# NERSC/swin_v2_weather

Hardware: AMD Instinct MI355X
Metric: ERA5 samples/sec (73x721x1440) swin_73var depth12 (higher is better)
Workload: dtype bf16

## Files before the change

include/swv2.h:

```cpp
#ifndef SWV2_H
#define SWV2_H
#include <stddef.h>
#include <stdint.h>

#ifdef __cplusplus
extern "C" {
#endif

#define SWV2_VERSION 113

enum {
    SWV2_OK = 0,
    SWV2_ERR_INVALID = -1,
    SWV2_ERR_UNSUPPORTED = -2,
    SWV2_ERR_LAUNCH = -3
};

int swv2_version(void);
const char* swv2_last_error(void);

int swv2_attn_geometry(int L, int head_dim, int* Lp, int* DP);

int swv2_attn_fwd_regime(int L, int head_dim, int has_bias, int dbg);

#define SWV2_ATTN_FIRST_GEN 16
#define SWV2_ATTN_PLAIN_STATS 8192
#define SWV2_ATTN_BWD_TWO_PHASE 32

typedef struct swv2_attn_args {
    const void* qkvh;
    const float* logit_scale;
    const float* bias;
    const void* bias_pack;
    void* oh;
    float* lse;
    const void* doh;
    const float* rnorm;
    void* dqkvh;
    float* dlogit_scale;
    float* dbias;
    int Bw, heads, L, head_dim;
    int nwh, nww;
    int mask_thr;
    int max_chunks;
    int dbg;
    void* dbias_ws;
    size_t dbias_ws_bytes;
    int dbias_partials;
} swv2_attn_args;

#define SWV2_ATTN_K_D256 0
#define SWV2_ATTN_K_FWD3 1
#define SWV2_ATTN_K_FWD3W 2
#define SWV2_ATTN_K_FWD3B 3
#define SWV2_ATTN_K_WIDE 4
#define SWV2_ATTN_K_STREAM 5
#define SWV2_ATTN_K_FIRST_GEN 6
typedef struct swv2_attn_kernel_t {
    int family;
    int Lp, DP;
    int LT, DK;
    int LFIX;
    int regime;
    int aug;
    int bias_lds;
    int qg;
} swv2_attn_kernel_t;
int swv2_attn_fwd_kernel(const swv2_attn_args* a, swv2_attn_kernel_t* out);
int swv2_attn_bwd_kernel(const swv2_attn_args* a, swv2_attn_kernel_t* out);

size_t swv2_attn_dbias_ws_bytes(int heads, int L, int max_chunks);

int swv2_attn_bias_chunks(int Bw);

size_t swv2_attn_pack_bias_bytes(int heads, int L);
int swv2_attn_pack_bias(const float* bias, int heads, int L, void* out, void* stream);
int swv2_attn_pack_bias_multi(const float* bias, int ntab, int heads, int L, void* out, void* stream);

int swv2_attn_fwd(const swv2_attn_args* a, void* stream);
int swv2_attn_bwd(const swv2_attn_args* a, void* stream);


enum swv2_operand_kind {
    SWV2_OP_F32 = 0,
    SWV2_OP_BF16 = 1,
    SWV2_OP_BF16_GELU = 2,
    SWV2_OP_HEADS = 3,
    SWV2_OP_PATCH = 4,
    SWV2_OP_MERGE_LN = 5,
    SWV2_OP_BF16_CSCALE = 6
};

typedef struct swv2_operand {
    int kind;
    const void* ptr;
    const int32_t* rowidx;
    const float* aux0;
    const float* aux1;
    const float* aux2;
    const float* aux3;
    long ld;
    int rows, cols;
    int p[4];
} swv2_operand;

enum swv2_epilogue_kind {
    SWV2_EPI_BF16 = 0,
    SWV2_EPI_F32 = 1,
    SWV2_EPI_QKV_HEADS = 2,
    SWV2_EPI_GELU_GRAD = 3,
    SWV2_EPI_UNPATCH = 4,
    SWV2_EPI_HEADS = 5,
    SWV2_EPI_F32_ACC = 6,
    SWV2_EPI_BF16_GELU = 7,
    SWV2_EPI_UNPATCH_LOSS = 8
};

typedef struct swv2_epilogue {
    int kind;
    void* out;
    const float* bias;
    const void* aux;
    float* aux_out;
    const int32_t* rowidx;
    long ld;
    int p[5];
    const float* loss_tar;
    const float* loss_qw;
    float* loss_part;
    void* loss_resid;
    int q[3];
} swv2_epilogue;

int swv2_linear(const swv2_operand* a, const void* w_bf16, const swv2_epilogue* e, int N, void* stream);

#define SWV2_LINEAR_RESIDENT_QKV128 0
#define SWV2_LINEAR_RESIDENT_QKV192X3 1
#define SWV2_LINEAR_RESIDENT_DX128 2
#define SWV2_LINEAR_WIDE_DMA 3
#define SWV2_LINEAR_WIDE 4
#define SWV2_LINEAR_TILE64 5
#define SWV2_LINEAR_TILE128 6
int swv2_linear_kernel(const swv2_operand* a, const swv2_epilogue* e, int N);

int swv2_linear_wgrad(const swv2_operand* dy, const swv2_operand* x, float* dW, float* db, const int32_t* nmap,
                      const int32_t* kmap, int ldw, int splits, void* stream);
size_t swv2_linear_wgrad_ws_bytes(int M, int N, int K, int splits);
int swv2_linear_wgrad_ws(const swv2_operand* dy, const swv2_operand* x, float* dW, float* db, const int32_t* nmap,
                         const int32_t* kmap, int ldw, int splits, void* ws, size_t ws_bytes, void* stream);
#define SWV2_WGRAD_WIDE 0
#define SWV2_WGRAD_TILE 1
int swv2_linear_wgrad_kernel(const swv2_operand* dy, const swv2_operand* x, int splits, size_t ws_bytes);

typedef struct swv2_wgrad_item {
    swv2_operand dy, x;
    float* dW;
    float* db;
    const int32_t* nmap;
    const int32_t* kmap;
    int ldw;
} swv2_wgrad_item;
size_t swv2_block_wgrad_ws_bytes(int C, int hidden, int heads_dp, int slices);
int swv2_block_wgrad(const swv2_wgrad_item* items4, int slices, void* ws, size_t ws_bytes, void* stream);
#define SWV2_BLOCK_WGRAD_SLAB 0
#define SWV2_BLOCK_WGRAD_GROUPED 1
int swv2_block_wgrad_kernel(const swv2_wgrad_item* items4, int slices, size_t ws_bytes);

int swv2_qk_normalize(void* qkvh_bf16, float* rnorm, int Bw, int heads, int Lp, int L, int DP, void* stream);

int swv2_prep_weight(const float* w, int rows, int cols, int transpose, const int32_t* row_map, int out_rows,
                     const int32_t* col_map, int out_cols, void* out_bf16, void* stream);

typedef struct swv2_prep_item {
    const float* w;
    int rows, cols, transpose;
    const int32_t* row_map;
    int out_rows;
    const int32_t* col_map;
    int out_cols;
    void* out;
    int out_f32;
} swv2_prep_item;
int swv2_prep_chunk(void);
int swv2_prep_item_chunks(int out_rows, int out_cols, int transpose);
int swv2_prep_multi(const swv2_prep_item* items_dev, const int* chunks_dev, int n_chunks, void* stream);

#define SWV2_LN_BWD_MAX_BLOCKS 512
typedef struct swv2_ln_args {
    const void* a;
    const float* res;
    const float* gamma;
    const float* beta;
    const float* scale;
    const int32_t* rowidx;
    float* y;
    float* mean;
    float* rstd;
    const float* dy;
    void* da;
    float* dgamma;
    float* dbeta;
    float* ws;
    int M, C, res_mod, rows_per_sample;
    float eps;
} swv2_ln_args;

int swv2_ln_residual_fwd(const swv2_ln_args* a, void* stream);
int swv2_ln_residual_bwd(const swv2_ln_args* a, void* stream);

int swv2_batch_sum(const float* in, float* out, int B, long n, int accumulate, void* stream);

int swv2_merge_stats(const float* x, float* mean, float* rstd, int B, int H, int W, int C, float eps, void* stream);
int swv2_merge_ln_bwd(const float* x, const void* dn_bf16, const float* gamma, const float* mean, const float* rstd,
                      float* dx, float* dgamma, float* dbeta, int B, int H, int W, int C, void* stream);

size_t swv2_loss_ws_bytes(int planes, int H, int W);
int swv2_loss_sums(const float* prd, const float* tar, const float* quad_w, float* sums, int BC, int H, int W, void* ws, size_t ws_bytes,
                   void* stream);
int swv2_loss_grad(const float* prd, const float* tar, const float* quad_w, const float* coef, float* dprd, int BC, int H,
                   int W, void* stream);
#define SWV2_LOSS_PART_SLICES 8
#define SWV2_LOSS_GROUP_ROWS 32
#define SWV2_LOSS_DUMP_BYTES 2048
#define SWV2_LOSS_RESID_PITCH(N) (((N) + 63) / 64 * 64)
int swv2_loss_part_reduce(const float* part, int M, int T, int B, int Cout, int Ct, int coff, float* sums, void* stream);
int swv2_loss_resid_to_image(const void* resid, const float* coef, const float* add, float* out, int B, int Cout, int H, int W, int Cs, int Cadd,
                             void* stream);
int swv2_loss_finalize(const float* sums, int layers, const float* chw, int BC, int C, int absolute, int squared, float* loss, float* coef,
                       void* stream);

int swv2_adam_step(float* p, const float* g, float* m, float* v, long n, float lr, float beta1, float beta2, float eps,
                   int step, float grad_inv_scale, void* stream);

typedef struct swv2_adam_item {
    float* p;
    const float* g;
    float* m;
    float* v;
    long n;
} swv2_adam_item;
int swv2_adam_chunk(void);
int swv2_adam_multi(const swv2_adam_item* items_dev, const int* chunks_dev, int n_chunks, float lr, float beta1, float beta2,
                    float eps, int step, float grad_inv_scale, void* stream);

typedef struct swv2_lamb_item {
    float* p;
    const float* g;
    float* m;
    float* v;
    long n;
    long chunk0;
} swv2_lamb_item;
#define SWV2_LAMB_SUM_DEPTH 64
#define SWV2_LAMB_ADAMW 1
#define SWV2_LAMB_BIAS_CORRECTION 2
#define SWV2_LAMB_GRAD_AVERAGING 4
#define SWV2_LAMB_NVLAMB 8
#define SWV2_LAMB_WS_GNORM2 0
#define SWV2_LAMB_WS_CLIP 1
#define SWV2_LAMB_WS_BC1 2
#define SWV2_LAMB_WS_BC2 3
#define SWV2_LAMB_WS_ITEM(i) (4 + 4 * (i))
int swv2_lamb_chunk(void);
size_t swv2_lamb_ws_bytes(int n_items, int n_chunks);
int swv2_lamb_grad_norm(const swv2_lamb_item* items_dev, const int* chunks_dev, int n_items, int n_chunks, float grad_inv_scale, void* ws,
                        size_t ws_bytes, void* stream);
int swv2_lamb_multi(const swv2_lamb_item* items_dev, const int* chunks_dev, int n_items, int n_chunks, int item_lo, int item_hi,
                    int chunk_lo, int chunk_hi, float lr, float beta1, float beta2, float eps, float weight_decay, float grad_inv_scale,
                    float max_grad_norm, int step, int flags, const float* extra_gnorm2, void* ws, size_t ws_bytes, void* stream);

int swv2_score_slices(int planes, int H, int W);
size_t swv2_score_ws_bytes(int planes, int H, int W);
int swv2_score_sums(const float* prd, long prd_bstride, const float* tar, long tar_bstride, const float* clim, const float* w, int B, int C,
                    int H, int W, void* ws, size_t ws_bytes, void* stream);
int swv2_score_finalize(const void* ws, size_t ws_bytes, int B, int C, int H, int W, const float* scale, float* sums, float* rmse, float* acc,
                        float* rmse_mean, float* acc_mean, void* stream);

int swv2_stats_slices(int C, int H, int W);
size_t swv2_stats_ws_bytes(int C, int H, int W);
int swv2_stats_accumulate(const float* slab, const float* prev, const double* pivot, double* tsum, void* part, size_t part_bytes, int C, int H,
                          int W, int first, void* stream);
int swv2_stats_finalize(const void* part, size_t part_bytes, const double* tsum, const double* pivot, int C, int H, int W, long T,
                        double* folded, float* time_means, void* stream);

size_t swv2_quantile_ws_bytes(int planes, int H, int W, int K);
int swv2_plane_order_stats(const float* x, long bstride, int B, int C, int H, int W, const int* ranks, int K, float* out, int* nan_count,
                           void* ws, size_t ws_bytes, void* stream);

size_t swv2_ens_ws_bytes(int planes, int H, int W, int M);
int swv2_ens_sums(const float* ens, long ens_mstride, long ens_bstride, const float* tar, long tar_bstride, const float* w, int M, int B, int C,
                  int H, int W, void* ws, size_t ws_bytes, void* stream);
int swv2_ens_finalize(const void* ws, size_t ws_bytes, int M, int B, int C, int H, int W, const float* scale, float* sums, int* hist,
                      float* ens_rmse, float* spread, float* crps, float* fair_crps, float* means, void* stream);

size_t swv2_l1_ws_bytes(int planes, int H, int W);
int swv2_l1_sums(const float* prd, long prd_bstride, const float* tar, long tar_bstride, const float* w, int B, int C, int H, int W, void* ws,
                 size_t ws_bytes, void* stream);
int swv2_l1_finalize(const void* ws, size_t ws_bytes, int B, int C, int H, int W, const float* chw, int absolute, float* sums, float* loss,
                     float* coef, void* stream);
int swv2_l1_grad(const float* prd, const float* tar, const float* quad_w, const float* coef, float* dprd, int BC, int H, int W, void* stream);

size_t swv2_sht_ws_bytes(int planes, int lmax, int mmax);
int swv2_sht_power(const float* table, const float* X, float* power, float* coeffs, int planes, int nlat, int lmax, int mmax, void* ws,
                   size_t ws_bytes, void* stream);
int swv2_sht_adjoint(const float* table, const float* coeffs, const float* gpower, float* dX, int planes, int nlat, int lmax, int mmax,
                     void* stream);
int swv2_sht_repack(const float* src, float* dst, int planes, int nlat, int mmax, float scale, int backward, void* stream);
int swv2_sht_synth(const float* table, const float* rweights, const float* coeffs, const float* response, int response_stride, float scale_m0,
                   float scale_m, float* S, int planes, int nlat, int lmax, int mmax, int nlon, void* stream);

int swv2_era5_select_normalize(const float* raw, float* out, const int* chan, const float* mean, const float* stdv, int B, int S,
                               int Csel, int Craw, int Hraw, int Wraw, int H, int W, int Cout_total, int coff, void* stream);
int swv2_era5_zenith(float* out, const float* sun, int B, int nz, int H, int W, int Cout_total, int coff, void* stream);
int swv2_era5_static(const float* stat, float* out, int B, int Cs, int H, int W, int Cout_total, int coff, void* stream);

int swv2_era5_select_normalize_i16(const int16_t* raw, float* out, const int* chan, const float* mean, const float* stdv, const float* offset,
                                   const float* scale, const int* slab_row, int B, int S, int Csel, int Craw, int Hraw, int Wraw, int H, int W,
                                   int Cout_total, int coff, void* stream);
int swv2_era5_unpack_i16(const int16_t* raw, float* out, const float* offset, const float* scale, int C, int H, int W, void* stream);
int swv2_era5_pack_i16(const float* slab, int16_t* out, const float* offset, const float* scale, int C, int H, int W, void* stream);
size_t swv2_pack_range_ws_bytes(int C, int H, int W);
int swv2_pack_range(const float* slab, int C, int H, int W, int first, float* range, int64_t* missing, void* ws, size_t ws_bytes, void* stream);

typedef struct {
    const void* oh;
    const void* wp;
    const float* bp;
    const float* gamma; const float* beta; const float* scale;
    const int32_t* rowidx;
    const float* x;
    void* a1; float* mean; float* rstd;
    float* y;
    int Bw, Lp, heads, C, rows_per_sample;
    float eps;
} swv2_proj_ln_args;
typedef struct {
    const float* dy;
    const void* a1; const float* mean; const float* rstd; const float* gamma; const float* scale;
    const int32_t* rowidx;
    const void* wpt;
    void* da1;
    void* doh;
    float* dgamma; float* dbeta; float* ws;
    int Bw, Lp, heads, C, rows_per_sample;
} swv2_proj_ln_bwd_args;
int swv2_proj_ln_supported(int C, int heads, int head_pad);
size_t swv2_proj_ln_bwd_ws_floats(int Mw, int C);
int swv2_proj_ln_fwd(const swv2_proj_ln_args* a, void* stream);
int swv2_proj_ln_bwd(const swv2_proj_ln_bwd_args* a, void* stream);

typedef struct {
    const float* x;
    const void* w1;
    const float* b1;
    const void* w2;
    const float* b2;
    const float* gamma;
    const float* beta;
    const float* scale;
    void* hpre;
    void* a2;
    float* mean;
    float* rstd;
    float* y;
    int M, C, hidden, rows_per_sample;
    float eps;
} swv2_mlp_args;
int swv2_mlp_supported(int C, int hidden);
int swv2_mlp_recompute_supported(int C, int hidden);
int swv2_mlp_fwd(const swv2_mlp_args* a, void* stream);

typedef struct {
    const float* dy;
    const void* a2;
    const float* mean;
    const float* rstd;
    const float* gamma;
    const float* scale;
    const void* hpre;
    const void* w2t;
    const void* w1t;
    void* da2;
    void* dh;
    float* dx;
    float* dgamma;
    float* dbeta;
    float* ws;
    int M, C, hidden, rows_per_sample;
    const float* x;
    const void* w1;
    const float* b1;
} swv2_mlp_bwd_args;
size_t swv2_mlp_bwd_ws_floats(int M, int C);
int swv2_mlp_bwd(const swv2_mlp_bwd_args* a, void* stream);

int swv2_cpb_fwd(const float* w1, const float* b1, const float* w2, const float* b2, const void* keep_bf16, float* bias,
                 int wh, int ww, int heads, int hidden, float drop_p, void* stream);
int swv2_cpb_bwd(const float* dbias, const float* w1, const float* b1, const float* w2, const void* keep_bf16, float* dw1,
                 float* db1, float* dw2, float* db2, int wh, int ww, int heads, int hidden, float drop_p, void* stream);
size_t swv2_cpb_bwd_ws_bytes(int wh, int ww, int heads, int hidden);
int swv2_cpb_bwd_ws(const float* dbias, const float* w1, const float* b1, const float* w2, const void* keep_bf16, float* dw1,
                    float* db1, float* dw2, float* db2, int wh, int ww, int heads, int hidden, float drop_p, void* ws,
                    size_t ws_bytes, void* stream);

int swv2_cpb_fwd_multi(const float* const* params_dev, int nblk, const uint32_t* keep_bits, float* bias, int wh, int ww, int heads,
                       int hidden, float drop_p, void* stream);
size_t swv2_cpb_bwd_multi_ws_bytes(int nblk, int wh, int ww, int heads, int hidden);
int swv2_cpb_bwd_multi(const float* dbias_tables, int nchunk, const float* const* params_dev, int nblk, const uint32_t* keep_bits,
                       float* grads, int wh, int ww, int heads, int hidden, float drop_p, void* ws, size_t ws_bytes, void* stream);

typedef struct swv2_block_desc {
    int B, T, C, heads, head_dim, hidden, L, Lp, DP, nwh, nww, mask_thr;
    const int32_t* rowidx;
    const int32_t* qkv_map;
    const int32_t* proj_map;
    const float *logit_scale, *qkv_b_pad, *proj_b, *n1_w, *n1_b, *fc1_b, *fc2_b, *n2_w, *n2_b;
    const void *w_qkv, *w_proj, *w_fc1, *w_fc2;
    const void *w_qkvt, *w_projt, *w_fc1t, *w_fc2t;
    const float* x;
    const float* bias;
    void* bias_pack;
    const float* dp1;
    const float* dp2;
    void* qkvh;  float* rnorm; void* oh; float* lse; void* a1; float* mean1; float* rstd1; float* x1;
    void* hpre;  void* hact;   void* a2; float* mean2; float* rstd2;
    float* x2;
    const float* dx2;
    void *da2, *dh, *da1, *doh, *dqkvh;
    float* dx1;
    float* ln_ws;
    float* dx;
    float *d_logit_scale, *d_bias, *d_qkv_w, *d_qkv_b, *d_proj_w, *d_proj_b, *d_n1_w, *d_n1_b, *d_fc1_w, *d_fc1_b,
          *d_fc2_w, *d_fc2_b, *d_n2_w, *d_n2_b;
    int wgrad_splits;
    int ev_kernel;
    void* ev_start;
    void* ev_stop;
    int fuse_proj_ln;
    int fuse_mlp;
    void* wgrad_ws;
    size_t wgrad_ws_bytes;
    int wgrad_group;
    void* grad_zero;
    size_t grad_zero_bytes;
    size_t ln_ws_floats;
    int bias_prepacked;
    float* dbias_part;
    size_t dbias_part_bytes;
} swv2_block_desc;

enum swv2_block_step {
    SWV2_STEP_RNORM_ZERO = 1,
    SWV2_STEP_QKV,
    SWV2_STEP_QK_NORMALIZE,
    SWV2_STEP_PACK_BIAS,
    SWV2_STEP_ATTN_FWD,
    SWV2_STEP_PROJ, SWV2_STEP_LN1_FWD,
    SWV2_STEP_PROJ_LN_FWD,
    SWV2_STEP_FC1, SWV2_STEP_FC2, SWV2_STEP_LN2_FWD,
    SWV2_STEP_MLP_FWD,
    SWV2_STEP_LN2_BWD, SWV2_STEP_WGRAD_FC2, SWV2_STEP_DH, SWV2_STEP_WGRAD_FC1, SWV2_STEP_DX1,
    SWV2_STEP_MLP_BWD,
    SWV2_STEP_LN1_BWD,
    SWV2_STEP_PROJ_LN_BWD,
    SWV2_STEP_WGRAD_PROJ, SWV2_STEP_DOH, SWV2_STEP_ATTN_BWD, SWV2_STEP_WGRAD_QKV, SWV2_STEP_DX,
    SWV2_STEP_LN_FOLD,
    SWV2_STEP_WGRAD_GROUP,
    SWV2_STEP_COUNT
};
#define SWV2_BLOCK_MAX_STEPS 12
enum { SWV2_DBIAS_NONE = 0,
       SWV2_DBIAS_ATOMICS = 1,
       SWV2_DBIAS_WGRAD_WS = 2,
       SWV2_DBIAS_PART = 3 };
typedef struct swv2_block_plan_t {
    int mlp_fused;
    int proj_ln_fused;
    int ln_deferred;
    int wgrad_grouped;
    int wgrad_kernel;
    int grad_zero_in_kernel;
    int attn_fwd_chunks, attn_bwd_chunks;
    int dbias_dest;
    size_t need_hact_bytes;
    size_t need_ln_ws_floats;
    size_t need_wgrad_ws_bytes;
    int n_fwd, n_bwd;
    int fwd[SWV2_BLOCK_MAX_STEPS], bwd[SWV2_BLOCK_MAX_STEPS];
} swv2_block_plan_t;
int swv2_block_plan(const swv2_block_desc* d, swv2_block_plan_t* out);
int swv2_block_step_id(int step);
const char* swv2_block_step_name(int step);

int swv2_block_fwd(const swv2_block_desc* d, void* stream);
int swv2_block_bwd(const swv2_block_desc* d, void* stream);

#ifdef __cplusplus
}
#endif
#endif
```

swin_v2_weather_amd/_lib.py:

```python
from __future__ import annotations

import ctypes as C
import os
import subprocess
import threading

HERE = os.path.dirname(os.path.abspath(__file__))
CSRC = os.path.join(HERE, "csrc")
LIB_PATH = os.environ.get("SWV2_LIB") or os.path.join(HERE, "libswv2.so")
SOURCES = ["capi.hip", "attn.hip", "attn2.hip", "attn_bwd_stream.hip", "attn_wide.hip", "attn_d256.hip", "gemm.hip", "gemm_tn.hip", "gemm_tn_slab.hip", "rowops.hip", "lamb.hip", "block.hip", "cpb.hip", "mlp.hip", "proj_ln.hip", "dataio.hip", "packed.hip", "score.hip", "stats.hip", "quantile.hip", "ensemble.hip", "loss_l1.hip", "loss_l2.hip", "sht.hip"]

ABI_VERSION = 113

_lib = None
_lock = threading.Lock()


class Swv2Error(RuntimeError):
    pass


def build_library(force: bool = False, verbose: bool = False) -> str:
    import glob
    srcs = [os.path.join(CSRC, s) for s in SOURCES]
    deps = srcs + glob.glob(os.path.join(CSRC, "*.h")) + [os.path.join(HERE, "..", "include", "swv2.h")]
    if not force and os.path.exists(LIB_PATH) and all(os.path.getmtime(LIB_PATH) >= os.path.getmtime(d) for d in deps):
        return LIB_PATH
    hipcc = os.environ.get("HIPCC", "/opt/rocm/bin/hipcc")
    objs, procs = [], []
    os.makedirs(os.path.join(HERE, "build"), exist_ok=True)
    for s in srcs:
        o = os.path.join(HERE, "build", os.path.basename(s) + ".o")
        objs.append(o)
        cmd = [hipcc, "--offload-arch=gfx950", "-O3", "-std=c++17", "-fPIC", "-c", s, "-o", o]
        procs.append((cmd, subprocess.Popen(cmd, stdout=subprocess.PIPE, stderr=subprocess.STDOUT)))
    for cmd, p in procs:
        out, _ = p.communicate()
        if p.returncode != 0:
            raise Swv2Error("hipcc failed: %s\n%s" % (" ".join(cmd), out.decode()))
        if verbose and out:
            print(out.decode())
    cmd = [hipcc, "--offload-arch=gfx950", "-shared", "-fPIC", "-o", LIB_PATH] + objs
    r = subprocess.run(cmd, stdout=subprocess.PIPE, stderr=subprocess.STDOUT)
    if r.returncode != 0:
        raise Swv2Error("link failed: %s\n%s" % (" ".join(cmd), r.stdout.decode()))
    return LIB_PATH


def source_hash() -> str:
    import glob
    import hashlib
    h = hashlib.sha256()
    files = sorted(glob.glob(os.path.join(CSRC, "*"))) + [os.path.join(HERE, "..", "include", "swv2.h")]
    for f in files:
        if os.path.isfile(f):
            h.update(os.path.basename(f).encode())
            h.update(open(f, "rb").read())
    return h.hexdigest()[:16]


class AttnArgs(C.Structure):
    _fields_ = [("qkvh", C.c_void_p), ("logit_scale", C.c_void_p), ("bias", C.c_void_p), ("bias_pack", C.c_void_p), ("oh", C.c_void_p),
                ("lse", C.c_void_p), ("doh", C.c_void_p), ("rnorm", C.c_void_p), ("dqkvh", C.c_void_p),
                ("dlogit_scale", C.c_void_p), ("dbias", C.c_void_p),
                ("Bw", C.c_int), ("heads", C.c_int), ("L", C.c_int), ("head_dim", C.c_int),
                ("nwh", C.c_int), ("nww", C.c_int), ("mask_thr", C.c_int), ("max_chunks", C.c_int), ("dbg", C.c_int),
                ("dbias_ws", C.c_void_p), ("dbias_ws_bytes", C.c_size_t), ("dbias_partials", C.c_int)]


class AttnKernelInfo(C.Structure):
    _fields_ = [(n, C.c_int) for n in ("family", "Lp", "DP", "LT", "DK", "LFIX", "regime", "aug", "bias_lds", "qg")]


ATTN_K_D256, ATTN_K_FWD3, ATTN_K_FWD3W, ATTN_K_FWD3B, ATTN_K_WIDE, ATTN_K_STREAM, ATTN_K_FIRST_GEN = range(7)
ATTN_K_NAMES = ("D256", "FWD3", "FWD3W", "FWD3B", "WIDE", "STREAM", "FIRST_GEN")


class Operand(C.Structure):
    _fields_ = [("kind", C.c_int), ("ptr", C.c_void_p), ("rowidx", C.c_void_p), ("aux0", C.c_void_p),
                ("aux1", C.c_void_p), ("aux2", C.c_void_p), ("aux3", C.c_void_p), ("ld", C.c_long),
                ("rows", C.c_int), ("cols", C.c_int), ("p", C.c_int * 4)]


class PrepItem(C.Structure):
    _fields_ = [("w", C.c_void_p), ("rows", C.c_int), ("cols", C.c_int), ("transpose", C.c_int), ("row_map", C.c_void_p),
                ("out_rows", C.c_int), ("col_map", C.c_void_p), ("out_cols", C.c_int), ("out", C.c_void_p), ("out_f32", C.c_int)]


class AdamItem(C.Structure):
    _fields_ = [("p", C.c_void_p), ("g", C.c_void_p), ("m", C.c_void_p), ("v", C.c_void_p), ("n", C.c_long)]


class LambItem(C.Structure):
    _fields_ = [("p", C.c_void_p), ("g", C.c_void_p), ("m", C.c_void_p), ("v", C.c_void_p), ("n", C.c_long), ("chunk0", C.c_long)]


class WgradItem(C.Structure):
    _fields_ = [("dy", Operand), ("x", Operand), ("dW", C.c_void_p), ("db", C.c_void_p), ("nmap", C.c_void_p),
                ("kmap", C.c_void_p), ("ldw", C.c_int)]


class Epilogue(C.Structure):
    _fields_ = [("kind", C.c_int), ("out", C.c_void_p), ("bias", C.c_void_p), ("aux", C.c_void_p),
                ("aux_out", C.c_void_p), ("rowidx", C.c_void_p), ("ld", C.c_long), ("p", C.c_int * 5),
                ("loss_tar", C.c_void_p), ("loss_qw", C.c_void_p), ("loss_part", C.c_void_p),
                ("loss_resid", C.c_void_p),
                ("q", C.c_int * 3)]


class ProjLnArgs(C.Structure):
    _fields_ = [(n, C.c_void_p) for n in ("oh", "wp", "bp", "gamma", "beta", "scale", "rowidx", "x", "a1", "mean", "rstd", "y")] + \
               [(n, C.c_int) for n in ("Bw", "Lp", "heads", "C", "rows_per_sample")] + [("eps", C.c_float)]


class ProjLnBwdArgs(C.Structure):
    _fields_ = [(n, C.c_void_p) for n in ("dy", "a1", "mean", "rstd", "gamma", "scale", "rowidx", "wpt", "da1", "doh", "dgamma", "dbeta",
                                           "ws")] + [(n, C.c_int) for n in ("Bw", "Lp", "heads", "C", "rows_per_sample")]


class MlpArgs(C.Structure):
    _fields_ = [(n, C.c_void_p) for n in ("x", "w1", "b1", "w2", "b2", "gamma", "beta", "scale", "hpre", "a2", "mean", "rstd", "y")] + \
               [(n, C.c_int) for n in ("M", "C", "hidden", "rows_per_sample")] + [("eps", C.c_float)]


class MlpBwdArgs(C.Structure):
    _fields_ = [(n, C.c_void_p) for n in ("dy", "a2", "mean", "rstd", "gamma", "scale", "hpre", "w2t", "w1t", "da2", "dh", "dx",
                                           "dgamma", "dbeta", "ws")] + [(n, C.c_int) for n in ("M", "C", "hidden", "rows_per_sample")] + \
               [(n, C.c_void_p) for n in ("x", "w1", "b1")]


class LnArgs(C.Structure):
    _fields_ = [("a", C.c_void_p), ("res", C.c_void_p), ("gamma", C.c_void_p), ("beta", C.c_void_p),
                ("scale", C.c_void_p), ("rowidx", C.c_void_p), ("y", C.c_void_p), ("mean", C.c_void_p),
                ("rstd", C.c_void_p), ("dy", C.c_void_p), ("da", C.c_void_p), ("dgamma", C.c_void_p),
                ("dbeta", C.c_void_p), ("ws", C.c_void_p), ("M", C.c_int), ("C", C.c_int), ("res_mod", C.c_int),
                ("rows_per_sample", C.c_int), ("eps", C.c_float)]


LN_BWD_MAX_BLOCKS = 512
ATTN_FIRST_GEN, ATTN_PLAIN_STATS, ATTN_BWD_TWO_PHASE = 16, 8192, 32
LOSS_PART_SLICES = 8
LOSS_GROUP_ROWS = 32
LOSS_DUMP_BYTES = 2048
SHT_MRUN = 8


def loss_resid_pitch(n: int) -> int:
    return (n + 63) // 64 * 64
class BlockDesc(C.Structure):
    _fields_ = ([(n, C.c_int) for n in ("B", "T", "C", "heads", "head_dim", "hidden", "L", "Lp", "DP", "nwh", "nww", "mask_thr")] +
                [(n, C.c_void_p) for n in (
                    "rowidx", "qkv_map", "proj_map",
                    "logit_scale", "qkv_b_pad", "proj_b", "n1_w", "n1_b", "fc1_b", "fc2_b", "n2_w", "n2_b",
                    "w_qkv", "w_proj", "w_fc1", "w_fc2", "w_qkvt", "w_projt", "w_fc1t", "w_fc2t",
                    "x", "bias", "bias_pack", "dp1", "dp2",
                    "qkvh", "rnorm", "oh", "lse", "a1", "mean1", "rstd1", "x1", "hpre", "hact", "a2", "mean2", "rstd2", "x2",
                    "dx2", "da2", "dh", "da1", "doh", "dqkvh", "dx1", "ln_ws", "dx",
                    "d_logit_scale", "d_bias", "d_qkv_w", "d_qkv_b", "d_proj_w", "d_proj_b", "d_n1_w", "d_n1_b", "d_fc1_w",
                    "d_fc1_b", "d_fc2_w", "d_fc2_b", "d_n2_w", "d_n2_b")] +
                [("wgrad_splits", C.c_int), ("ev_kernel", C.c_int), ("ev_start", C.c_void_p), ("ev_stop", C.c_void_p),
                 ("fuse_proj_ln", C.c_int), ("fuse_mlp", C.c_int), ("wgrad_ws", C.c_void_p), ("wgrad_ws_bytes", C.c_size_t), ("wgrad_group", C.c_int), ("grad_zero", C.c_void_p),
                 ("grad_zero_bytes", C.c_size_t), ("ln_ws_floats", C.c_size_t),
                 ("bias_prepacked", C.c_int), ("dbias_part", C.c_void_p), ("dbias_part_bytes", C.c_size_t)])


LAMB_ADAMW, LAMB_BIAS_CORRECTION, LAMB_GRAD_AVERAGING, LAMB_NVLAMB = 1, 2, 4, 8
LAMB_SUM_DEPTH = 64
LAMB_WS_GNORM2, LAMB_WS_CLIP, LAMB_WS_BC1, LAMB_WS_BC2 = range(4)


def lamb_ws_item(i: int) -> int:
    return 4 + 4 * i


BLOCK_MAX_STEPS = 12
DBIAS_NONE, DBIAS_ATOMICS, DBIAS_WGRAD_WS, DBIAS_PART = range(4)


class BlockPlan(C.Structure):
    _fields_ = ([(n, C.c_int) for n in ("mlp_fused", "proj_ln_fused", "ln_deferred", "wgrad_grouped", "wgrad_kernel", "grad_zero_in_kernel",
                                        "attn_fwd_chunks", "attn_bwd_chunks", "dbias_dest")] +
                [(n, C.c_size_t) for n in ("need_hact_bytes", "need_ln_ws_floats", "need_wgrad_ws_bytes")] +
                [("n_fwd", C.c_int), ("n_bwd", C.c_int), ("fwd", C.c_int * BLOCK_MAX_STEPS), ("bwd", C.c_int * BLOCK_MAX_STEPS)])

    def steps(self, phase):
        lib = load()
        return [lib.swv2_block_step_name(s).decode() for s in getattr(self, phase)[:getattr(self, "n_" + phase)]]


def block_plan(desc: BlockDesc) -> BlockPlan:
    plan = BlockPlan()
    check(load().swv2_block_plan(C.byref(desc), C.byref(plan)), "swv2_block_plan")
    return plan


OP_F32, OP_BF16, OP_BF16_GELU, OP_HEADS, OP_PATCH, OP_MERGE_LN, OP_BF16_CSCALE = range(7)
EPI_BF16, EPI_F32, EPI_QKV_HEADS, EPI_GELU_GRAD, EPI_UNPATCH, EPI_HEADS, EPI_F32_ACC, EPI_BF16_GELU, EPI_UNPATCH_LOSS = range(9)
LINEAR_RESIDENT_QKV128, LINEAR_RESIDENT_QKV192X3, LINEAR_RESIDENT_DX128, LINEAR_WIDE_DMA, LINEAR_WIDE, LINEAR_TILE64, LINEAR_TILE128 = range(7)
LINEAR_WIDE_KERNELS, LINEAR_TILE_KERNELS = (LINEAR_WIDE_DMA, LINEAR_WIDE), (LINEAR_TILE64, LINEAR_TILE128)
WGRAD_WIDE, WGRAD_TILE = range(2)
BLOCK_WGRAD_SLAB, BLOCK_WGRAD_GROUPED = range(2)

_P, _I, _L, _F = C.c_void_p, C.c_int, C.c_long, C.c_float
SYMBOLS = {
    "swv2_version": (_I, []),
    "swv2_last_error": (C.c_char_p, []),
    "swv2_attn_geometry": (_I, [_I, _I, C.POINTER(_I), C.POINTER(_I)]),
    "swv2_attn_fwd_regime": (_I, [_I, _I, _I, _I]),
    "swv2_attn_fwd_kernel": (_I, [C.POINTER(AttnArgs), C.POINTER(AttnKernelInfo)]),
    "swv2_attn_bwd_kernel": (_I, [C.POINTER(AttnArgs), C.POINTER(AttnKernelInfo)]),
    "swv2_attn_pack_bias_bytes": (C.c_size_t, [_I, _I]),
    "swv2_attn_dbias_ws_bytes": (C.c_size_t, [_I, _I, _I]),
    "swv2_attn_pack_bias": (_I, [_P, _I, _I, _P, _P]),
    "swv2_attn_pack_bias_multi": (_I, [_P, _I, _I, _I, _P, _P]),
    "swv2_attn_bias_chunks": (_I, [_I]),
    "swv2_attn_fwd": (_I, [C.POINTER(AttnArgs), _P]),
    "swv2_attn_bwd": (_I, [C.POINTER(AttnArgs), _P]),
    "swv2_linear": (_I, [C.POINTER(Operand), _P, C.POINTER(Epilogue), _I, _P]),
    "swv2_linear_kernel": (_I, [C.POINTER(Operand), C.POINTER(Epilogue), _I]),
    "swv2_linear_wgrad_kernel": (_I, [C.POINTER(Operand), C.POINTER(Operand), _I, C.c_size_t]),
    "swv2_block_wgrad_kernel": (_I, [C.POINTER(WgradItem), _I, C.c_size_t]),
    "swv2_linear_wgrad": (_I, [C.POINTER(Operand), C.POINTER(Operand), _P, _P, _P, _P, _I, _I, _P]),
    "swv2_linear_wgrad_ws_bytes": (C.c_size_t, [_I, _I, _I, _I]),
    "swv2_qk_normalize": (_I, [_P, _P, _I, _I, _I, _I, _I, _P]),
    "swv2_block_wgrad_ws_bytes": (C.c_size_t, [_I, _I, _I, _I]),
    "swv2_block_wgrad": (_I, [C.POINTER(WgradItem), _I, _P, C.c_size_t, _P]),
    "swv2_linear_wgrad_ws": (_I, [C.POINTER(Operand), C.POINTER(Operand), _P, _P, _P, _P, _I, _I, _P, C.c_size_t, _P]),
    "swv2_prep_weight": (_I, [_P, _I, _I, _I, _P, _I, _P, _I, _P, _P]),
    "swv2_ln_residual_fwd": (_I, [C.POINTER(LnArgs), _P]),
    "swv2_ln_residual_bwd": (_I, [C.POINTER(LnArgs), _P]),
    "swv2_batch_sum": (_I, [_P, _P, _I, _L, _I, _P]),
    "swv2_merge_stats": (_I, [_P, _P, _P, _I, _I, _I, _I, _F, _P]),
    "swv2_merge_ln_bwd": (_I, [_P, _P, _P, _P, _P, _P, _P, _P, _I, _I, _I, _I, _P]),
    "swv2_loss_ws_bytes": (C.c_size_t, [_I, _I, _I]),
    "swv2_loss_sums": (_I, [_P, _P, _P, _P, _I, _I, _I, _P, C.c_size_t, _P]),
    "swv2_loss_grad": (_I, [_P, _P, _P, _P, _P, _I, _I, _I, _P]),
    "swv2_loss_part_reduce": (_I, [_P, _I, _I, _I, _I, _I, _I, _P, _P]),
    "swv2_loss_resid_to_image": (_I, [_P, _P, _P, _P, _I, _I, _I, _I, _I, _I, _P]),
    "swv2_loss_finalize": (_I, [_P, _I, _P, _I, _I, _I, _I, _P, _P, _P]),
    "swv2_prep_chunk": (_I, []),
    "swv2_prep_item_chunks": (_I, [_I, _I, _I]),
    "swv2_prep_multi": (_I, [_P, _P, _I, _P]),
    "swv2_adam_chunk": (_I, []),
    "swv2_adam_multi": (_I, [_P, _P, _I, _F, _F, _F, _F, _I, _F, _P]),
    "swv2_adam_step": (_I, [_P, _P, _P, _P, _L, _F, _F, _F, _F, _I, _F, _P]),
    "swv2_lamb_chunk": (_I, []),
    "swv2_lamb_ws_bytes": (C.c_size_t, [_I, _I]),
    "swv2_lamb_grad_norm": (_I, [_P, _P, _I, _I, _F, _P, C.c_size_t, _P]),
    "swv2_lamb_multi": (_I, [_P, _P, _I, _I, _I, _I, _I, _I, _F, _F, _F, _F, _F, _F, _F, _I, _I, _P, _P, C.c_size_t, _P]),
    "swv2_score_slices": (_I, [_I, _I, _I]),
    "swv2_score_ws_bytes": (C.c_size_t, [_I, _I, _I]),
    "swv2_score_sums": (_I, [_P, _L, _P, _L, _P, _P, _I, _I, _I, _I, _P, C.c_size_t, _P]),
    "swv2_score_finalize": (_I, [_P, C.c_size_t, _I, _I, _I, _I, _P, _P, _P, _P, _P, _P, _P]),
    "swv2_stats_slices": (_I, [_I, _I, _I]),
    "swv2_stats_ws_bytes": (C.c_size_t, [_I, _I, _I]),
    "swv2_stats_accumulate": (_I, [_P, _P, _P, _P, _P, C.c_size_t, _I, _I, _I, _I, _P]),
    "swv2_stats_finalize": (_I, [_P, C.c_size_t, _P, _P, _I, _I, _I, _L, _P, _P, _P]),
    "swv2_quantile_ws_bytes": (C.c_size_t, [_I, _I, _I, _I]),
    "swv2_plane_order_stats": (_I, [_P, _L, _I, _I, _I, _I, _P, _I, _P, _P, _P, C.c_size_t, _P]),
    "swv2_ens_ws_bytes": (C.c_size_t, [_I, _I, _I, _I]),
    "swv2_ens_sums": (_I, [_P, _L, _L, _P, _L, _P, _I, _I, _I, _I, _I, _P, C.c_size_t, _P]),
    "swv2_ens_finalize": (_I, [_P, C.c_size_t, _I, _I, _I, _I, _I, _P, _P, _P, _P, _P, _P, _P, _P, _P]),
    "swv2_l1_ws_bytes": (C.c_size_t, [_I, _I, _I]),
    "swv2_l1_sums": (_I, [_P, _L, _P, _L, _P, _I, _I, _I, _I, _P, C.c_size_t, _P]),
    "swv2_l1_finalize": (_I, [_P, C.c_size_t, _I, _I, _I, _I, _P, _I, _P, _P, _P, _P]),
    "swv2_l1_grad": (_I, [_P, _P, _P, _P, _P, _I, _I, _I, _P]),
    "swv2_sht_ws_bytes": (C.c_size_t, [_I, _I, _I]),
    "swv2_sht_power": (_I, [_P, _P, _P, _P, _I, _I, _I, _I, _P, C.c_size_t, _P]),
    "swv2_sht_adjoint": (_I, [_P, _P, _P, _P, _I, _I, _I, _I, _P]),
    "swv2_sht_repack": (_I, [_P, _P, _I, _I, _I, _F, _I, _P]),
    "swv2_sht_synth": (_I, [_P, _P, _P, _P, _I, _F, _F, _P, _I, _I, _I, _I, _I, _P]),
    "swv2_era5_select_normalize": (_I, [_P, _P, _P, _P, _P] + [_I] * 10 + [_P]),
    "swv2_era5_zenith": (_I, [_P, _P, _I, _I, _I, _I, _I, _I, _P]),
    "swv2_era5_static": (_I, [_P, _P, _I, _I, _I, _I, _I, _I, _P]),
    "swv2_era5_select_normalize_i16": (_I, [_P] * 8 + [_I] * 10 + [_P]),
    "swv2_era5_unpack_i16": (_I, [_P, _P, _P, _P, _I, _I, _I, _P]),
    "swv2_era5_pack_i16": (_I, [_P, _P, _P, _P, _I, _I, _I, _P]),
    "swv2_pack_range_ws_bytes": (C.c_size_t, [_I, _I, _I]),
    "swv2_pack_range": (_I, [_P, _I, _I, _I, _I, _P, _P, _P, C.c_size_t, _P]),
    "swv2_proj_ln_supported": (_I, [_I, _I, _I]),
    "swv2_proj_ln_bwd_ws_floats": (C.c_size_t, [_I, _I]),
    "swv2_proj_ln_fwd": (_I, [C.POINTER(ProjLnArgs), _P]),
    "swv2_proj_ln_bwd": (_I, [C.POINTER(ProjLnBwdArgs), _P]),
    "swv2_mlp_supported": (_I, [_I, _I]),
    "swv2_mlp_recompute_supported": (_I, [_I, _I]),
    "swv2_mlp_fwd": (_I, [C.POINTER(MlpArgs), _P]),
    "swv2_mlp_bwd_ws_floats": (C.c_size_t, [_I, _I]),
    "swv2_mlp_bwd": (_I, [C.POINTER(MlpBwdArgs), _P]),
    "swv2_cpb_fwd": (_I, [_P, _P, _P, _P, _P, _P, _I, _I, _I, _I, _F, _P]),
    "swv2_cpb_bwd": (_I, [_P, _P, _P, _P, _P, _P, _P, _P, _P, _I, _I, _I, _I, _F, _P]),
    "swv2_cpb_bwd_ws": (_I, [_P, _P, _P, _P, _P, _P, _P, _P, _P, _I, _I, _I, _I, _F, _P, C.c_size_t, _P]),
    "swv2_cpb_bwd_ws_bytes": (C.c_size_t, [_I, _I, _I, _I]),
    "swv2_cpb_fwd_multi": (_I, [_P, _I, _P, _P, _I, _I, _I, _I, _F, _P]),
    "swv2_cpb_bwd_multi_ws_bytes": (C.c_size_t, [_I, _I, _I, _I, _I]),
    "swv2_cpb_bwd_multi": (_I, [_P, _I, _P, _I, _P, _P, _I, _I, _I, _I, _F, _P, C.c_size_t, _P]),
    "swv2_block_plan": (_I, [C.POINTER(BlockDesc), C.POINTER(BlockPlan)]),
    "swv2_block_step_id": (_I, [_I]),
    "swv2_block_step_name": (C.c_char_p, [_I]),
    "swv2_block_fwd": (_I, [C.POINTER(BlockDesc), _P]),
    "swv2_block_bwd": (_I, [C.POINTER(BlockDesc), _P]),
}


def load() -> C.CDLL:
    global _lib
    if _lib is not None:
        return _lib
    with _lock:
        if _lib is None:
            if not os.path.exists(LIB_PATH):
                raise Swv2Error(f"{LIB_PATH} not found: run `python -c 'import __graft_entry__ as g; g.build()'` "
                                "(the HIP library is required; there is no fallback path)")
            import torch
            lib = C.CDLL(LIB_PATH)
            for name, (res, args) in SYMBOLS.items():
                fn = getattr(lib, name)
                fn.restype, fn.argtypes = res, args
            got = lib.swv2_version()
            if got != ABI_VERSION:
                raise Swv2Error(f"{LIB_PATH} reports ABI revision {got}, this binding mirrors revision {ABI_VERSION} of include/swv2.h: "
                                "rebuild the library (python -c 'import __graft_entry__ as g; g.build()')")
            _lib = lib
    return _lib


def check(rc: int, what: str = "") -> None:
    if rc != 0:
        msg = load().swv2_last_error()
        raise Swv2Error(f"{what} failed with code {rc}: {msg.decode() if msg else ''}")
```

swin_v2_weather_amd/csrc/block.hip:

```cpp
#include "common.h"

namespace {

swv2_operand op(int kind, const void* p, int rows, int cols, long ld, const int32_t* rowidx = nullptr) {
    swv2_operand o = {};
    o.kind = kind; o.ptr = p; o.rowidx = rowidx; o.ld = ld; o.rows = rows; o.cols = cols;
    return o;
}
swv2_operand op_heads(const void* p, int Bw, int heads, int parts, int Lp, int DP) {
    swv2_operand o = op(SWV2_OP_HEADS, p, Bw * Lp, parts * heads * DP, parts);
    o.p[0] = heads; o.p[2] = Lp; o.p[3] = DP;
    return o;
}
swv2_epilogue epi(int kind, void* out, long ld, const float* bias = nullptr, const void* aux = nullptr,
                  float* aux_out = nullptr, const int32_t* rowidx = nullptr) {
    swv2_epilogue e = {};
    e.kind = kind; e.out = out; e.ld = ld; e.bias = bias; e.aux = aux; e.aux_out = aux_out; e.rowidx = rowidx;
    return e;
}
swv2_attn_args attn(const swv2_block_desc* d, int max_chunks) {
    swv2_attn_args a = {};
    a.qkvh = d->qkvh; a.logit_scale = d->logit_scale; a.bias = d->bias; a.bias_pack = d->bias ? d->bias_pack : nullptr;
    a.oh = d->oh; a.lse = d->lse;
    a.Bw = d->B * d->nwh * d->nww; a.heads = d->heads; a.L = d->L; a.head_dim = d->head_dim; a.nwh = d->nwh; a.nww = d->nww;
    a.mask_thr = d->mask_thr; a.max_chunks = max_chunks;
    return a;
}
void wgrad_items(const swv2_block_desc* d, bool fused, swv2_wgrad_item it[4]) {
    const int BT = d->B * d->T, Bw = d->B * d->nwh * d->nww, Mw = Bw * d->Lp, C = d->C, h = d->heads, hid = d->hidden;
    it[0].dy = op(SWV2_OP_BF16, d->da2, BT, C, C);
    it[0].x = fused ? op(SWV2_OP_BF16_GELU, d->hpre, BT, hid, hid) : op(SWV2_OP_BF16, d->hact, BT, hid, hid);
    it[0].dW = d->d_fc2_w; it[0].db = d->d_fc2_b; it[0].ldw = hid;
    it[1].dy = op(SWV2_OP_BF16, d->dh, BT, hid, hid); it[1].x = op(SWV2_OP_F32, d->x1, BT, C, C);
    it[1].dW = d->d_fc1_w; it[1].db = d->d_fc1_b; it[1].ldw = C;
    it[2].dy = op(SWV2_OP_BF16, d->da1, Mw, C, C); it[2].x = op_heads(d->oh, Bw, h, 1, d->Lp, d->DP);
    it[2].dW = d->d_proj_w; it[2].db = d->d_proj_b; it[2].kmap = d->proj_map; it[2].ldw = C;
    it[3].dy = op_heads(d->dqkvh, Bw, h, 3, d->Lp, d->DP); it[3].x = op(SWV2_OP_F32, d->x, Mw, C, C, d->rowidx);
    it[3].dW = d->d_qkv_w; it[3].db = d->d_qkv_b; it[3].nmap = d->qkv_map; it[3].ldw = C;
}
#define TRY(x) do { int rc_ = (x); if (rc_) return rc_; } while (0)

const struct { int id; const char* name; } STEPS[SWV2_STEP_COUNT] = {
    {0, "end"},
    {0, "rnorm_zero"}, {1, "qkv"}, {0, "qk_normalize"}, {0, "pack_bias"}, {2, "attn_fwd"}, {3, "proj"}, {4, "ln1_fwd"}, {3, "proj_ln_fwd"},
    {5, "fc1"}, {6, "fc2"}, {7, "ln2_fwd"}, {5, "mlp_fwd"},
    {11, "ln2_bwd"}, {12, "wgrad_fc2"}, {13, "dh"}, {14, "wgrad_fc1"}, {15, "dx1"}, {13, "mlp_bwd"}, {16, "ln1_bwd"}, {16, "proj_ln_bwd"},
    {17, "wgrad_proj"}, {18, "doh"}, {19, "attn_bwd"}, {20, "wgrad_qkv"}, {21, "dx"}, {0, "ln_fold"}, {22, "wgrad_group"},
};
static_assert(SWV2_STEP_WGRAD_GROUP + 1 == SWV2_STEP_COUNT && SWV2_STEP_MLP_FWD == 12 && SWV2_STEP_LN2_BWD == 13, "STEPS follows enum swv2_block_step");

#define LAUNCH(step, x)                                                                                     \
    do {                                                                                                    \
        const bool t_ = d->ev_kernel == STEPS[step].id && d->ev_start && d->ev_stop;                         \
        if (t_) (void)hipEventRecord((hipEvent_t)d->ev_start, (hipStream_t)st);                             \
        TRY(x);                                                                                             \
        if (t_) (void)hipEventRecord((hipEvent_t)d->ev_stop, (hipStream_t)st);                              \
    } while (0)

int plan_block(const swv2_block_desc* d, swv2_block_plan_t* p) {
    SWV2_CHECK_ARG(d && p, "swv2_block_plan: null descriptor or plan");
    SWV2_CHECK_ARG(d->B > 0 && d->T > 0 && d->C > 0 && d->heads > 0 && d->hidden > 0 && d->Lp > 0 && d->DP > 0 && d->nwh > 0 && d->nww > 0,
                   "swv2_block_plan: non-positive geometry");
    *p = {};
    const int BT = d->B * d->T, Bw = d->B * d->nwh * d->nww, Mw = Bw * d->Lp, C = d->C, h = d->heads, hid = d->hidden;
    const int sp = d->wgrad_splits > 0 ? d->wgrad_splits : 64;
    const size_t ws_bytes = d->wgrad_ws ? d->wgrad_ws_bytes : 0;
    const size_t ln_pair = swv2_mlp_bwd_ws_floats(BT, C) + swv2_proj_ln_bwd_ws_floats(Mw, C);
    p->need_ln_ws_floats = std::max((size_t)SWV2_LN_BWD_MAX_BLOCKS * 2 * C, ln_pair);
    p->need_wgrad_ws_bytes = d->wgrad_group ? swv2_block_wgrad_ws_bytes(C, hid, h * d->DP, 0) : 0;
    const int prod[4][3] = {{BT, C, hid}, {BT, hid, C}, {Mw, C, h * d->DP}, {Mw, 3 * h * d->DP, C}};
    for (const auto& q : prod)
        p->need_wgrad_ws_bytes = std::max(p->need_wgrad_ws_bytes, swv2_linear_wgrad_ws_bytes(q[0], q[1], q[2], sp));

    p->mlp_fused = d->fuse_mlp && swv2_mlp_supported(C, hid);
    p->proj_ln_fused = d->fuse_proj_ln && swv2_proj_ln_supported(C, h, d->DP);
    p->need_hact_bytes = p->mlp_fused ? 0 : (size_t)BT * hid * 2;
    p->ln_deferred = p->mlp_fused && p->proj_ln_fused && d->ln_ws_floats >= ln_pair;
    p->wgrad_grouped = d->wgrad_group && p->mlp_fused && d->wgrad_ws && ws_bytes >= swv2_block_wgrad_ws_bytes(C, hid, h * d->DP, 0);
    p->wgrad_kernel = -1;
    p->grad_zero_in_kernel = p->mlp_fused && d->grad_zero != nullptr;
    p->attn_fwd_chunks = d->bias ? 32 : 64;
    p->attn_bwd_chunks = 64;
    if (d->bias) {
        p->attn_bwd_chunks = swv2_attn_bias_chunks(Bw);
        p->dbias_dest = d->dbias_part ? SWV2_DBIAS_PART : ws_bytes ? SWV2_DBIAS_WGRAD_WS : SWV2_DBIAS_ATOMICS;
    } else if (d->Lp == 176 && h <= 256) {
        p->attn_bwd_chunks = 256 / h;
    }

    auto fwd = [&](int s) { p->fwd[p->n_fwd++] = s; };
    auto bwd = [&](int s) { p->bwd[p->n_bwd++] = s; };
    const bool wide = d->DP > 64;
    if (wide) fwd(SWV2_STEP_RNORM_ZERO);
    fwd(SWV2_STEP_QKV);
    if (wide) fwd(SWV2_STEP_QK_NORMALIZE);
    if (d->bias && d->bias_pack && !d->bias_prepacked) fwd(SWV2_STEP_PACK_BIAS);
    fwd(SWV2_STEP_ATTN_FWD);
    if (p->proj_ln_fused) fwd(SWV2_STEP_PROJ_LN_FWD);
    else { fwd(SWV2_STEP_PROJ); fwd(SWV2_STEP_LN1_FWD); }
    if (p->mlp_fused) fwd(SWV2_STEP_MLP_FWD);
    else { fwd(SWV2_STEP_FC1); fwd(SWV2_STEP_FC2); fwd(SWV2_STEP_LN2_FWD); }

    const bool single = !p->wgrad_grouped;
    if (p->mlp_fused) {
        bwd(SWV2_STEP_MLP_BWD);
        if (single) { bwd(SWV2_STEP_WGRAD_FC2); bwd(SWV2_STEP_WGRAD_FC1); }
    } else {
        bwd(SWV2_STEP_LN2_BWD); bwd(SWV2_STEP_WGRAD_FC2); bwd(SWV2_STEP_DH); bwd(SWV2_STEP_WGRAD_FC1); bwd(SWV2_STEP_DX1);
    }
    bwd(p->proj_ln_fused ? SWV2_STEP_PROJ_LN_BWD : SWV2_STEP_LN1_BWD);
    if (single) bwd(SWV2_STEP_WGRAD_PROJ);
    if (!p->proj_ln_fused) bwd(SWV2_STEP_DOH);
    bwd(SWV2_STEP_ATTN_BWD);
    if (single) bwd(SWV2_STEP_WGRAD_QKV);
    bwd(SWV2_STEP_DX);
    if (p->ln_deferred && single) bwd(SWV2_STEP_LN_FOLD);
    if (p->wgrad_grouped) bwd(SWV2_STEP_WGRAD_GROUP);
    return SWV2_OK;
}

}

extern "C" int swv2_block_step_id(int step) { return step > 0 && step < SWV2_STEP_COUNT ? STEPS[step].id : -1; }
extern "C" const char* swv2_block_step_name(int step) { return step > 0 && step < SWV2_STEP_COUNT ? STEPS[step].name : nullptr; }

extern "C" int swv2_block_plan(const swv2_block_desc* d, swv2_block_plan_t* p) {
    TRY(plan_block(d, p));
    if (p->wgrad_grouped) {
        swv2_wgrad_item it[4] = {};
        wgrad_items(d, true, it);
        p->wgrad_kernel = swv2_block_wgrad_kernel(it, 0, d->wgrad_ws_bytes);
    }
    return SWV2_OK;
}

extern "C" int swv2_block_fwd(const swv2_block_desc* d, void* st) {
    SWV2_CHECK_ARG(d && d->x && d->x2 && d->qkvh && d->rowidx, "swv2_block_fwd: null descriptor field");
    swv2_block_plan_t p;
    TRY(plan_block(d, &p));
    SWV2_CHECK_ARG(d->hact || !p.need_hact_bytes, "swv2_block_fwd: the separate MLP kernels need hact (swv2_block_plan: need_hact_bytes)");
    const int BT = d->B * d->T, Bw = d->B * d->nwh * d->nww, Mw = Bw * d->Lp, C = d->C, h = d->heads, hid = d->hidden;
    for (int i = 0; i < p.n_fwd; ++i) switch (p.fwd[i]) {
    case SWV2_STEP_RNORM_ZERO:
        if (hipMemsetAsync(d->rnorm, 0, (size_t)Bw * h * 2 * d->Lp * sizeof(float), (hipStream_t)st) != hipSuccess) {
            swv2_set_error("swv2_block_fwd: hipMemsetAsync(rnorm) failed");
            return SWV2_ERR_LAUNCH;
        }
        break;
    case SWV2_STEP_QKV: {
        swv2_operand a = op(SWV2_OP_F32, d->x, Mw, C, C, d->rowidx);
        swv2_epilogue e = epi(SWV2_EPI_QKV_HEADS, d->qkvh, 0, d->qkv_b_pad, nullptr, d->rnorm);
        e.p[0] = h; e.p[2] = d->Lp; e.p[3] = d->DP; e.p[4] = d->L;
        LAUNCH(SWV2_STEP_QKV, swv2_linear(&a, d->w_qkv, &e, 3 * h * d->DP, st));
    } break;
    case SWV2_STEP_QK_NORMALIZE: TRY(swv2_qk_normalize(d->qkvh, (float*)d->rnorm, Bw, h, d->Lp, d->L, d->DP, st)); break;
    case SWV2_STEP_PACK_BIAS: TRY(swv2_attn_pack_bias(d->bias, h, d->L, d->bias_pack, st)); break;
    case SWV2_STEP_ATTN_FWD: {
        swv2_attn_args a = attn(d, p.attn_fwd_chunks);
        LAUNCH(SWV2_STEP_ATTN_FWD, swv2_attn_fwd(&a, st));
    } break;
    case SWV2_STEP_PROJ_LN_FWD: {
        swv2_proj_ln_args m = {};
        m.oh = d->oh; m.wp = d->w_proj; m.bp = d->proj_b; m.gamma = d->n1_w; m.beta = d->n1_b; m.scale = d->dp1; m.rowidx = d->rowidx;
        m.x = d->x; m.a1 = d->a1; m.mean = d->mean1; m.rstd = d->rstd1; m.y = d->x1; m.Bw = Bw; m.Lp = d->Lp; m.heads = h; m.C = C;
        m.rows_per_sample = d->T; m.eps = 1e-5f;
        LAUNCH(SWV2_STEP_PROJ_LN_FWD, swv2_proj_ln_fwd(&m, st));
    } break;
    case SWV2_STEP_PROJ: {
        swv2_operand a = op_heads(d->oh, Bw, h, 1, d->Lp, d->DP);
        swv2_epilogue e = epi(SWV2_EPI_BF16, d->a1, C, d->proj_b);
        LAUNCH(SWV2_STEP_PROJ, swv2_linear(&a, d->w_proj, &e, C, st));
    } break;
    case SWV2_STEP_LN1_FWD: {
        swv2_ln_args l = {};
        l.a = d->a1; l.res = d->x; l.gamma = d->n1_w; l.beta = d->n1_b; l.scale = d->dp1; l.rowidx = d->rowidx; l.y = d->x1;
        l.mean = d->mean1; l.rstd = d->rstd1; l.M = Mw; l.C = C; l.res_mod = 0; l.rows_per_sample = d->T; l.eps = 1e-5f;
        LAUNCH(SWV2_STEP_LN1_FWD, swv2_ln_residual_fwd(&l, st));
    } break;
    case SWV2_STEP_MLP_FWD: {
        swv2_mlp_args m = {};
        m.x = d->x1; m.w1 = d->w_fc1; m.b1 = d->fc1_b; m.w2 = d->w_fc2; m.b2 = d->fc2_b; m.gamma = d->n2_w; m.beta = d->n2_b;
        m.scale = d->dp2; m.hpre = d->hpre; m.a2 = d->a2; m.mean = d->mean2; m.rstd = d->rstd2; m.y = d->x2;
        m.M = BT; m.C = C; m.hidden = hid; m.rows_per_sample = d->T; m.eps = 1e-5f;
        LAUNCH(SWV2_STEP_MLP_FWD, swv2_mlp_fwd(&m, st));
    } break;
    case SWV2_STEP_FC1: {
        swv2_operand a = op(SWV2_OP_F32, d->x1, BT, C, C);
        swv2_epilogue e = epi(SWV2_EPI_BF16_GELU, d->hpre, hid, d->fc1_b, nullptr, (float*)d->hact);
        LAUNCH(SWV2_STEP_FC1, swv2_linear(&a, d->w_fc1, &e, hid, st));
    } break;
    case SWV2_STEP_FC2: {
        swv2_operand a = op(SWV2_OP_BF16, d->hact, BT, hid, hid);
        swv2_epilogue e = epi(SWV2_EPI_BF16, d->a2, C, d->fc2_b);
        LAUNCH(SWV2_STEP_FC2, swv2_linear(&a, d->w_fc2, &e, C, st));
    } break;
    case SWV2_STEP_LN2_FWD: {
        swv2_ln_args l = {};
        l.a = d->a2; l.res = d->x1; l.gamma = d->n2_w; l.beta = d->n2_b; l.scale = d->dp2; l.y = d->x2; l.mean = d->mean2;
        l.rstd = d->rstd2; l.M = BT; l.C = C; l.res_mod = 0; l.rows_per_sample = d->T; l.eps = 1e-5f;
        LAUNCH(SWV2_STEP_LN2_FWD, swv2_ln_residual_fwd(&l, st));
    } break;
    }
    return SWV2_OK;
}

extern "C" int swv2_block_bwd(const swv2_block_desc* d, void* st) {
    SWV2_CHECK_ARG(d && d->dx2 && d->dx && d->da2 && d->dh && d->dx1 && d->da1 && d->doh && d->dqkvh && d->ln_ws,
                   "swv2_block_bwd: null descriptor field");
    swv2_block_plan_t p;
    TRY(plan_block(d, &p));
    SWV2_CHECK_ARG(d->hact || !p.need_hact_bytes, "swv2_block_bwd: the separate MLP kernels need hact (swv2_block_plan: need_hact_bytes)");
    const int BT = d->B * d->T, Bw = d->B * d->nwh * d->nww, Mw = Bw * d->Lp, C = d->C, h = d->heads, hid = d->hidden;
    const int sp = d->wgrad_splits > 0 ? d->wgrad_splits : 64;
    swv2_wgrad_item it[4] = {};
    wgrad_items(d, p.mlp_fused, it);
    float* const ln1_ws = p.ln_deferred ? d->ln_ws + swv2_mlp_bwd_ws_floats(BT, C) : d->ln_ws;
    int n_ln1 = 0, n_ln2 = 0;
    for (int i = 0; i < p.n_bwd; ++i) switch (const int s = p.bwd[i]; s) {
    case SWV2_STEP_MLP_BWD: {
        swv2_mlp_bwd_args m = {};
        m.dy = d->dx2; m.a2 = d->a2; m.mean = d->mean2; m.rstd = d->rstd2; m.gamma = d->n2_w; m.scale = d->dp2; m.hpre = d->hpre;
        m.w2t = d->w_fc2t; m.w1t = d->w_fc1t; m.da2 = d->da2; m.dh = d->dh; m.dx = d->dx1; m.dgamma = d->d_n2_w;
        m.dbeta = d->d_n2_b; m.ws = d->ln_ws; m.M = BT; m.C = C; m.hidden = hid; m.rows_per_sample = d->T;
        LAUNCH(SWV2_STEP_MLP_BWD, swv2_mlp_bwd_impl(&m, st, p.ln_deferred ? &n_ln2 : nullptr, p.grad_zero_in_kernel ? (float*)d->grad_zero : nullptr,
                                                    (long)(d->grad_zero_bytes / 4)));
    } break;
    case SWV2_STEP_LN2_BWD: {
        swv2_ln_args l = {};
        l.a = d->a2; l.dy = d->dx2; l.gamma = d->n2_w; l.scale = d->dp2; l.mean = d->mean2; l.rstd = d->rstd2; l.da = d->da2;
        l.dgamma = d->d_n2_w; l.dbeta = d->d_n2_b; l.ws = d->ln_ws; l.M = BT; l.C = C; l.rows_per_sample = d->T;
        LAUNCH(SWV2_STEP_LN2_BWD, swv2_ln_residual_bwd(&l, st));
    } break;
    case SWV2_STEP_WGRAD_FC2: case SWV2_STEP_WGRAD_FC1: case SWV2_STEP_WGRAD_PROJ: case SWV2_STEP_WGRAD_QKV: {
        const swv2_wgrad_item& w = it[s == SWV2_STEP_WGRAD_FC2 ? 0 : s == SWV2_STEP_WGRAD_FC1 ? 1 : s == SWV2_STEP_WGRAD_PROJ ? 2 : 3];
        LAUNCH(s, swv2_linear_wgrad_ws(&w.dy, &w.x, w.dW, w.db, w.nmap, w.kmap, w.ldw, sp, d->wgrad_ws, d->wgrad_ws_bytes, st));
    } break;
    case SWV2_STEP_DH: {
        swv2_epilogue e = epi(SWV2_EPI_GELU_GRAD, d->dh, hid, nullptr, d->hpre);
        LAUNCH(SWV2_STEP_DH, swv2_linear(&it[0].dy, d->w_fc2t, &e, hid, st));
    } break;
    case SWV2_STEP_DX1: {
        swv2_epilogue e = epi(SWV2_EPI_F32, d->dx1, C, nullptr, d->dx2);
        LAUNCH(SWV2_STEP_DX1, swv2_linear(&it[1].dy, d->w_fc1t, &e, C, st));
    } break;
    case SWV2_STEP_PROJ_LN_BWD: {
        swv2_proj_ln_bwd_args m = {};
        m.dy = d->dx1; m.a1 = d->a1; m.mean = d->mean1; m.rstd = d->rstd1; m.gamma = d->n1_w; m.scale = d->dp1; m.rowidx = d->rowidx;
        m.wpt = d->w_projt; m.da1 = d->da1; m.doh = d->doh; m.dgamma = d->d_n1_w; m.dbeta = d->d_n1_b; m.ws = ln1_ws;
        m.Bw = Bw; m.Lp = d->Lp; m.heads = h; m.C = C; m.rows_per_sample = d->T;
        LAUNCH(SWV2_STEP_PROJ_LN_BWD, swv2_proj_ln_bwd_impl(&m, st, p.ln_deferred ? &n_ln1 : nullptr));
    } break;
    case SWV2_STEP_LN1_BWD: {
        swv2_ln_args l = {};
        l.a = d->a1; l.dy = d->dx1; l.gamma = d->n1_w; l.scale = d->dp1; l.rowidx = d->rowidx; l.mean = d->mean1; l.rstd = d->rstd1;
        l.da = d->da1; l.dgamma = d->d_n1_w; l.dbeta = d->d_n1_b; l.ws = d->ln_ws; l.M = Mw; l.C = C; l.rows_per_sample = d->T;
        LAUNCH(SWV2_STEP_LN1_BWD, swv2_ln_residual_bwd(&l, st));
    } break;
    case SWV2_STEP_DOH: {
        swv2_epilogue e = epi(SWV2_EPI_HEADS, d->doh, 0);
        e.p[0] = h; e.p[2] = d->Lp; e.p[3] = d->DP; e.p[4] = d->L;
        LAUNCH(SWV2_STEP_DOH, swv2_linear(&it[2].dy, d->w_projt, &e, h * d->DP, st));
    } break;
    case SWV2_STEP_ATTN_BWD: {
        swv2_attn_args a = attn(d, p.attn_bwd_chunks);
        a.doh = d->doh; a.rnorm = d->rnorm; a.dqkvh = d->dqkvh; a.dlogit_scale = d->d_logit_scale; a.dbias = d->d_bias;
        if (p.dbias_dest == SWV2_DBIAS_PART) { a.dbias_ws = d->dbias_part; a.dbias_ws_bytes = d->dbias_part_bytes; a.dbias_partials = 1; }
        if (p.dbias_dest == SWV2_DBIAS_WGRAD_WS) { a.dbias_ws = d->wgrad_ws; a.dbias_ws_bytes = d->wgrad_ws_bytes; }
        LAUNCH(SWV2_STEP_ATTN_BWD, swv2_attn_bwd(&a, st));
    } break;
    case SWV2_STEP_DX: {
        swv2_epilogue e = epi(SWV2_EPI_F32, d->dx, C, nullptr, d->dx1, nullptr, d->rowidx);
        LAUNCH(SWV2_STEP_DX, swv2_linear(&it[3].dy, d->w_qkvt, &e, C, st));
    } break;
    case SWV2_STEP_LN_FOLD:
        swv2_launch_ln_partials_reduce2(d->ln_ws, d->d_n2_w, d->d_n2_b, n_ln2, ln1_ws, d->d_n1_w, d->d_n1_b, n_ln1, C, (hipStream_t)st);
        break;
    case SWV2_STEP_WGRAD_GROUP: {
        swv2_ln_partials lnp = {{d->ln_ws, ln1_ws}, {d->d_n2_w, d->d_n1_w}, {d->d_n2_b, d->d_n1_b}, {n_ln2, n_ln1}, C};
        LAUNCH(SWV2_STEP_WGRAD_GROUP, swv2_block_wgrad_ln(it, 0, d->wgrad_ws, d->wgrad_ws_bytes, p.ln_deferred ? &lnp : nullptr, st));
    } break;
    }
    return SWV2_OK;
}
```

swin_v2_weather_amd/csrc/gemm.hip:

```cpp
#include "common.h"

#include <cmath>
#include <cstdlib>
#include "gemm_common.h"

namespace {

constexpr int EP = 68;

struct EpiDesc {
    void* out;
    const float* bias;
    const void* aux;
    float* aux_out;
    const int32_t* rowidx;
    long ld;
    int M, N;
    int p0, p1, p2, p3, p4;
    uint32_t mg0, mg1, mg2;
    const float* loss_tar; const float* loss_qw; float* loss_part; uint16_t* loss_resid; int q0, q1, q2, q3;
};

enum { E_BF16 = 0, E_F32 = 1, E_QKV_HEADS = 2, E_GELU_GRAD = 3, E_UNPATCH = 4, E_HEADS = 5, E_F32_ACC = 6, E_BF16_GELU = 7,
       E_UNPATCH_LOSS = 8, E_UNPATCH_LOSS_SKIP = 9 };
// ... 638 lines not shown
    const int wr = wave >> 2, wc = wave & 3;
    const int xcd = blockIdx.x & 7, nper = gridDim.x >> 3, stages = K / 32;
    const uint32_t lds0 = (uint32_t)(uintptr_t)smem;
    const int drow = wave * 32 + (lane >> 2);
    int dkc[2];
#pragma unroll
    for (int i = 0; i < 2; ++i) dkc[i] = (lane & 3) ^ ((0 - ((drow + 16 * i) >> 2)) & 3);
    struct Tile { int m_base, n_base; uint32_t boff[2], aoff[2]; };
    auto make_tile = [&](int mt, int nt) {
        Tile t;
        t.m_base = mt * WBM; t.n_base = nt * WBN;
#pragma unroll
        for (int i = 0; i < 2; ++i) {
            const int row = drow + 16 * i;
            t.boff[i] = 2u * (uint32_t)(min(t.n_base + row, N - 1) * K + dkc[i] * 8);
            t.aoff[i] = AK == A_BF16 ? 2u * (uint32_t)(min(t.m_base + row, M - 1) * (int)al.d.ld + dkc[i] * 8) : 0u;
        }
        return t;
    };
    auto issue = [&](const Tile& tl, int t, int slot) {
        const uint32_t la = lds0 + (uint32_t)(slot * WSTG * 2) + (uint32_t)(wave * 2048), lb = la + WBM * 32 * 2;
#pragma unroll
        for (int i = 0; i < 2; ++i) dma_x4(Wb + t * 32, tl.boff[i], lb + 1024 * i);
        if constexpr (AK == A_BF16) {
#pragma unroll
            for (int i = 0; i < 2; ++i) dma_x4((const uint16_t*)al.d.ptr + t * 32, tl.aoff[i], la + 1024 * i);
        } else {
#pragma unroll
            for (int i = 0; i < 2; ++i)
                dma_x4(al.d.ptr, 2u * al.elem_off(min(tl.m_base + drow + 16 * i, M - 1), t * 32 + dkc[i] * 8), la + 1024 * i);
        }
    };
    int v = blockIdx.x >> 3, mt = 0, nt = 0;
    while (v < vmax && !wide_tile(xcd, v, mtiles, ntn, mt, nt)) v += nper;
    if (v >= vmax) return;
    Tile cur = make_tile(mt, nt);
    issue(cur, 0, 0); issue(cur, 1, 1); issue(cur, 2, 2);
    asm volatile("s_waitcnt vmcnt(8)" ::: "memory");
    __builtin_amdgcn_s_barrier();
    if (wr == 1) __builtin_amdgcn_s_barrier();
    for (;;) {
        int v2 = v + nper, mt2 = 0, nt2 = 0;
        while (v2 < vmax && !wide_tile(xcd, v2, mtiles, ntn, mt2, nt2)) v2 += nper;
        const bool has_next = v2 < vmax;
        const Tile nxt = has_next ? make_tile(mt2, nt2) : cur;
        f32x4 acc[8][4];
#pragma unroll
        for (int i = 0; i < 8; ++i)
#pragma unroll
            for (int j = 0; j < 4; ++j) acc[i][j] = (f32x4){0.f, 0.f, 0.f, 0.f};
        for (int t = 0; t < stages; ++t) {
            if (t + 3 < stages) issue(cur, t + 3, (t + 3) & 3);
            else issue(nxt, has_next ? t + 3 - stages : stages - 1, (t + 3) & 3);
            const uint16_t* As = smem + (t & 3) * WSTG;
            const uint16_t* Bs = As + WBM * 32;
            bf16x8 af[8], bf[4];
#pragma unroll
            for (int j = 0; j < 4; ++j) bf[j] = *(const bf16x8*)(Bs + swz32(wc * 64 + j * 16 + fr, g));
#pragma unroll
            for (int i = 0; i < 8; ++i) af[i] = *(const bf16x8*)(As + swz32(wr * 128 + i * 16 + fr, g));
            asm volatile("s_waitcnt vmcnt(8)" ::: "memory");
            asm volatile("s_waitcnt lgkmcnt(0)" ::: "memory");
            __builtin_amdgcn_sched_barrier(0);
            __builtin_amdgcn_s_barrier();
            __builtin_amdgcn_sched_barrier(0);
            __builtin_amdgcn_s_setprio(1);
#pragma unroll
            for (int i = 0; i < 8; ++i)
#pragma unroll
                for (int j = 0; j < 4; ++j) acc[i][j] = mfma32(af[i], bf[j], acc[i][j]);
            __builtin_amdgcn_s_setprio(0);
            __builtin_amdgcn_sched_barrier(0);
            __builtin_amdgcn_s_barrier();
            __builtin_amdgcn_sched_barrier(0);
        }
        if (wr == 0) __builtin_amdgcn_s_barrier();
        __builtin_amdgcn_sched_barrier(0);
        {
            float* st = (float*)(smem + 3 * WSTG) + wave * 16 * EP;
            if (cur.n_base + wc * 64 < N) wide_epilogue<EK>(ep, acc, st, cur.m_base + wr * 128, cur.n_base + wc * 64, lane);
        }
        asm volatile("s_waitcnt lgkmcnt(0)" ::: "memory");
        __builtin_amdgcn_sched_barrier(0);
        __builtin_amdgcn_s_barrier();
        if (wr == 1) __builtin_amdgcn_s_barrier();
        __builtin_amdgcn_sched_barrier(0);
        if (!has_next) break;
        cur = nxt; v = v2;
    }
    if (wr == 0) __builtin_amdgcn_s_barrier();
}

__device__ __forceinline__ int tn_pchunk(int row, int c) { return ((((c >> 1) ^ (row & 7)) << 1) | (c & 1)); }
template <int YK, int XK>
__global__ __launch_bounds__(WTH) void gemm_tn_wide_kernel(ALoad<YK> yl, ALoad<XK> xl, float* __restrict__ part, float* __restrict__ dbpart,
                                                           int M, int N, int K, int S, int wgs, int per_xcd) {
    static_assert((YK == A_BF16 || YK == A_HEADS) && (XK == A_BF16 || XK == A_HEADS), "raw bf16 operands");
    constexpr int SLABE = 32 * 256;
    __shared__ __attribute__((aligned(1024))) unsigned char smem_b[WSM_BYTES];
    uint16_t* const smem = (uint16_t*)smem_b;
    const int tid = threadIdx.x, lane = tid & 63, wave = __builtin_amdgcn_readfirstlane(tid >> 6);
    const int fr = lane & 15, g = lane >> 4;
    const int wr = wave >> 2, wc = wave & 3;
    const int w = (blockIdx.x & 7) * per_xcd + (blockIdx.x >> 3);
    if ((int)(blockIdx.x >> 3) >= per_xcd || w >= wgs) return;
    const int ntk = K / WBN, tiles = (N / WBM) * ntk;
    const int slice = w / tiles, tile = w - slice * tiles, tn = tile / ntk, tk = tile - tn * ntk;
    const int n_base = tn * WBM, k_base = tk * WBN;
    const int T = M / 32, t0 = (int)((long)slice * T / S), t1 = (int)((long)(slice + 1) * T / S), stages = t1 - t0;
    const uint32_t lds0 = (uint32_t)(uintptr_t)smem;
    int drw[2], dcl[2];
    uint32_t yoff[2], xoff[2];
#pragma unroll
    for (int i = 0; i < 2; ++i) {
        drw[i] = wave * 4 + 2 * i + (lane >> 5);
        dcl[i] = tn_pchunk(drw[i], lane & 31) * 8;
        yoff[i] = YK == A_BF16 ? 2u * (uint32_t)((t0 * 32 + drw[i]) * (int)yl.d.ld + n_base + dcl[i]) : 0u;
        xoff[i] = XK == A_BF16 ? 2u * (uint32_t)((t0 * 32 + drw[i]) * (int)xl.d.ld + k_base + dcl[i]) : 0u;
    }
    const long ystep = 32 * (long)yl.d.ld, xstep = 32 * (long)xl.d.ld;
    auto issue = [&](int t, int slot) {
        const uint32_t ly = lds0 + (uint32_t)(slot * WSTG * 2) + (uint32_t)(wave * 2048), lx = ly + SLABE * 2;
#pragma unroll
        for (int i = 0; i < 2; ++i) {
            if constexpr (YK == A_BF16) dma_x4((const uint16_t*)yl.d.ptr + t * ystep, yoff[i], ly + 1024 * i);
            else dma_x4(yl.d.ptr, 2u * yl.elem_off((t0 + t) * 32 + drw[i], n_base + dcl[i]), ly + 1024 * i);
        }
#pragma unroll
        for (int i = 0; i < 2; ++i) {
            if constexpr (XK == A_BF16) dma_x4((const uint16_t*)xl.d.ptr + t * xstep, xoff[i], lx + 1024 * i);
            else dma_x4(xl.d.ptr, 2u * xl.elem_off((t0 + t) * 32 + drw[i], k_base + dcl[i]), lx + 1024 * i);
        }
    };
    f32x4 acc[8][4];
#pragma unroll
    for (int i = 0; i < 8; ++i)
#pragma unroll
        for (int j = 0; j < 4; ++j) acc[i][j] = (f32x4){0.f, 0.f, 0.f, 0.f};
    auto trf = [&](const uint16_t* slab, int r0, int c0) -> bf16x4 {
        const int row = r0 + 4 * g + (fr >> 2), col = c0 + (fr & 3) * 4;
        return lds_tr_read(slab + row * 256 + tn_pchunk(row, col >> 3) * 8 + (col & 7));
    };
    float cs[8] = {0.f, 0.f, 0.f, 0.f, 0.f, 0.f, 0.f, 0.f};
    const int cs_off = (tid >> 5) * 256 + tn_pchunk(tid >> 5, tid & 31) * 8;
    const bool want_db = dbpart != nullptr;

    if (stages > 0) {
        issue(0, 0); issue(min(1, stages - 1), 1); issue(min(2, stages - 1), 2);
        asm volatile("s_waitcnt vmcnt(8)" ::: "memory");
        __builtin_amdgcn_s_barrier();
        if (wr == 1) __builtin_amdgcn_s_barrier();
        for (int t = 0; t < stages; ++t) {
            issue(min(t + 3, stages - 1), (t + 3) & 3);
            const uint16_t* Ys = smem + (t & 3) * WSTG;
            const uint16_t* Xs = Ys + SLABE;
            bf16x8 af[8], bf[4];
#pragma unroll
            for (int j = 0; j < 4; ++j)
                bf[j] = __builtin_shufflevector(trf(Xs, 0, wc * 64 + 16 * j), trf(Xs, 16, wc * 64 + 16 * j), 0, 1, 2, 3, 4, 5, 6, 7);
#pragma unroll
            for (int i = 0; i < 8; ++i)
                af[i] = __builtin_shufflevector(trf(Ys, 0, wr * 128 + 16 * i), trf(Ys, 16, wr * 128 + 16 * i), 0, 1, 2, 3, 4, 5, 6, 7);
            if (want_db && ((t0 + t) % ntk) == tk) {
                const uint4 a = *(const uint4*)(Ys + cs_off), b = *(const uint4*)(Ys + cs_off + 16 * 256);
                float va[8], vb[8];
                unpack8(a, va); unpack8(b, vb);
#pragma unroll
                for (int e = 0; e < 8; ++e) cs[e] += va[e] + vb[e];
            }
            asm volatile("s_waitcnt vmcnt(8)" ::: "memory");
            asm volatile("s_waitcnt lgkmcnt(0)" ::: "memory");
            __builtin_amdgcn_sched_barrier(0);
            __builtin_amdgcn_s_barrier();
            __builtin_amdgcn_sched_barrier(0);
            __builtin_amdgcn_s_setprio(1);
#pragma unroll
            for (int i = 0; i < 8; ++i)
#pragma unroll
                for (int j = 0; j < 4; ++j) acc[i][j] = mfma32(af[i], bf[j], acc[i][j]);
            __builtin_amdgcn_s_setprio(0);
            __builtin_amdgcn_sched_barrier(0);
            __builtin_amdgcn_s_barrier();
            __builtin_amdgcn_sched_barrier(0);
        }
        if (wr == 0) __builtin_amdgcn_s_barrier();
        asm volatile("s_waitcnt vmcnt(0)" ::: "memory");
    }
    __syncthreads();
    Epi<E_F32> ep;
    ep.d.out = part + (size_t)slice * N * K; ep.d.bias = nullptr; ep.d.aux = nullptr; ep.d.aux_out = nullptr; ep.d.rowidx = nullptr;
    ep.d.ld = K; ep.d.M = N; ep.d.N = K;
    wide_epilogue<E_F32>(ep, acc, (float*)smem + wave * 16 * EP, n_base + wr * 128, k_base + wc * 64, lane);
    if (want_db) {
        __syncthreads();
        float* red = (float*)smem;
#pragma unroll
        for (int e = 0; e < 8; ++e) red[(tid >> 5) * 256 + (tid & 31) * 8 + e] = cs[e];
        __syncthreads();
        if (tid < 256) {
            float sum = 0.f;
#pragma unroll
            for (int r = 0; r < 16; ++r) sum += red[r * 256 + tid];
            dbpart[((size_t)slice * ntk + tk) * N + n_base + tid] = sum;
        }
    }
}

template <int AK, int EK>
__global__ __launch_bounds__(WTH) void gemm_nt_wide_kernel(ALoad<AK> al, const uint16_t* __restrict__ Wb, Epi<EK> ep,
                                                           int M, int N, int K, int mtiles, int ntn) {
    static_assert(!ALoad<AK>::ROW_FASTEST, "row-major staging map only");
    constexpr int TILE = (WBM + WBN) * BK;
    __shared__ __attribute__((aligned(1024))) uint16_t smem[2 * TILE];
    static_assert(2 * TILE * 2 >= 8 * 16 * EP * 4, "the epilogue staging re-uses the tile buffers");
    const int tid = threadIdx.x, lane = tid & 63, wave = __builtin_amdgcn_readfirstlane(tid >> 6);
    const int fr = lane & 15, g = lane >> 4;
    const int wr = wave >> 2, wc = wave & 3;
    int mt, nt;
    if (!wide_tile(blockIdx.x & 7, blockIdx.x >> 3, mtiles, ntn, mt, nt)) return;
    const int m_base = mt * WBM, n_base = nt * WBN;
    const uint32_t lds0 = (uint32_t)(uintptr_t)smem;
    f32x4 acc[8][4];
#pragma unroll
    for (int i = 0; i < 8; ++i)
#pragma unroll
        for (int j = 0; j < 4; ++j) acc[i][j] = (f32x4){0.f, 0.f, 0.f, 0.f};
    {
        const int ksteps = K / BK;
        const int drow = wave * 32 + (lane >> 3);
        uint32_t boff[4];
#pragma unroll
        for (int i = 0; i < 4; ++i) {
            const int row = drow + 8 * i, kcl = (lane & 7) ^ ((row >> 1) & 7);
            boff[i] = 2u * (uint32_t)((n_base + row) * K + kcl * 8);
        }
        typename ALoad<AK>::Raw ra[4];
        int arow[4];
        uint32_t aok = 0;
        const int kc = tid & 7;
#pragma unroll
        for (int i = 0; i < 4; ++i) {
            const int src = al.row_of(m_base + (tid >> 3) + 64 * i);
            arow[i] = max(src, 0);
            aok |= (src >= 0 ? 1u : 0u) << i;
        }
        auto issue = [&](int s, int buf) {
            const uint32_t lb = lds0 + (uint32_t)(buf * TILE * 2) + (uint32_t)(wave * 4096) + WBM * BK * 2;
#pragma unroll
            for (int i = 0; i < 4; ++i) dma_x4(Wb + s * BK, boff[i], lb + 1024 * i);
#pragma unroll
            for (int i = 0; i < 4; ++i) ra[i] = al.raw_unc(arow[i], s * BK + kc * 8);
        };
        auto commit = [&](int buf) {
            uint16_t* As = smem + buf * TILE;
#pragma unroll
            for (int i = 0; i < 4; ++i) {
                uint4 v = al.cvt(ra[i]);
                if (!((aok >> i) & 1)) v = make_uint4(0, 0, 0, 0);
                *(uint4*)(As + swz((tid >> 3) + 64 * i, kc)) = v;
            }
        };
        auto compute = [&](int buf) {
            const uint16_t* As = smem + buf * TILE;
            const uint16_t* Bs = As + WBM * BK;
#pragma unroll
            for (int kk = 0; kk < 2; ++kk) {
                bf16x8 bf[4];
#pragma unroll
                for (int j = 0; j < 4; ++j) bf[j] = *(const bf16x8*)(Bs + swz(wc * 64 + j * 16 + fr, kk * 4 + g));
#pragma unroll
                for (int i = 0; i < 8; ++i) {
                    const bf16x8 af = *(const bf16x8*)(As + swz(wr * 128 + i * 16 + fr, kk * 4 + g));
#pragma unroll
                    for (int j = 0; j < 4; ++j) acc[i][j] = mfma32(af, bf[j], acc[i][j]);
                }
            }
        };
        issue(0, 0);
        asm volatile("s_waitcnt vmcnt(0)" ::: "memory");
        commit(0);
        __syncthreads();
        for (int s = 0; s + 1 < ksteps; ++s) {
            issue(s + 1, (s + 1) & 1);
            __builtin_amdgcn_sched_barrier(0);
            compute(s & 1);
            __builtin_amdgcn_sched_barrier(0);
            asm volatile("s_waitcnt vmcnt(0)" ::: "memory");
            commit((s + 1) & 1);
            __syncthreads();
        }
        compute((ksteps - 1) & 1);
        __syncthreads();
    }
    wide_epilogue<EK>(ep, acc, (float*)smem + wave * 16 * EP, m_base + wr * 128, n_base + wc * 64, lane);
}

#ifdef SWV2_RW_STAMPS
__device__ unsigned long long rw_stamps[256 * 8];
#define SWV2_STAMPS
#endif
#include "stamps.h"
__device__ __forceinline__ int swzk(int r, int kc, int K) { return r * K + ((kc ^ ((r >> 1) & 7)) << 3); }

template <int AK, int EK, int N, int K, int BMT, int HS = 16>
__global__ __launch_bounds__(512) void gemm_rw_kernel(ALoad<AK> al, const uint16_t* __restrict__ Wb, Epi<EK> ep, int M) {
    constexpr int NTH = 512, KC = K / 8;
    constexpr int ACH = BMT * KC / NTH;
    constexpr int RT = BMT / 64;
    constexpr int CT = N / 32;
    constexpr int WCH = N * KC / NTH;
    constexpr int A_BYTES = BMT * K * 2, ST_BYTES = 8 * 16 * EP * 4;
    constexpr int AS_BYTES = A_BYTES > ST_BYTES ? A_BYTES : ST_BYTES;
    static_assert(BMT * KC % NTH == 0 && N * KC % NTH == 0 && K % 64 == 0 && N % 64 == 0, "tile shapes");
    static_assert(N * K * 2 + AS_BYTES <= 160 * 1024, "LDS budget");
    __shared__ __attribute__((aligned(16))) uint16_t Ws[N * K];
    __shared__ __attribute__((aligned(16))) unsigned char as_raw[AS_BYTES];
    __shared__ __attribute__((aligned(16))) float bs[N];
    uint16_t* As = (uint16_t*)as_raw;
    float* stage_all = (float*)as_raw;

    const int tid = threadIdx.x, lane = tid & 63, wave = tid >> 6;
    const int fr = lane & 15, g = lane >> 4;
    const int wr = wave >> 1, wc = wave & 1;
    const int ntiles = (M + BMT - 1) / BMT;
    static_assert(EK != E_F32 || (RT == 1 && CT == 4), "the E_F32 prefetch below covers one 16 x 64 wave tile");
    for (int i = tid; i < N; i += NTH) bs[i] = ep.d.bias ? ep.d.bias[i] : 0.f;
    int erow_nxt = -1, erow_cur = -1;
    f32x4 aux_nxt[4], aux_cur[4];
    const int ecol = wc * (N / 2) + (lane & 3) * 16;

    typename ALoad<AK>::Raw ra[ACH];
    int arow[ACH];
    int erow_res = -1;
    auto crow = [&](int c) { return AK == A_HEADS ? ((c >> 1) & (BMT - 1)) : c / KC; };
    auto ccol = [&](int c) { return AK == A_HEADS ? (((c / (2 * BMT)) << 1) | (c & 1)) : c % KC; };
    static_assert(AK != A_HEADS || (BMT & (BMT - 1)) == 0, "head-major chunk map needs a power-of-two tile height");
    uint32_t ain = 0;
    uint32_t aok = 0;
    bool ein = false;
    auto resolve = [&](int t) {
        ain = 0;
#pragma unroll
        for (int i = 0; i < ACH; ++i) {
            const int c = tid + i * NTH, m = t * BMT + crow(c);
            const bool in = (t < ntiles) && (m < M);
            ain |= (uint32_t)in << i;
            if constexpr (AK == A_F32) arow[i] = al.d.rowidx[min(m, M - 1)];
            else arow[i] = min(m, M - 1);
        }
        if constexpr (EK == E_F32) {
            const int m = t * BMT + wr * 16 + (lane >> 2);
            ein = (t < ntiles) && (m < M);
            erow_res = ein ? ep.d.rowidx[m] : -1;
        }
    };
    auto issue = [&]() {
        aok = 0;
#pragma unroll
        for (int i = 0; i < ACH; ++i) {
            const int c = tid + i * NTH;
            const int r = ((ain >> i) & 1) ? arow[i] : -1;
            if constexpr (AK == A_HEADS) ra[i] = al.raw_at(r, ccol(c) * 8);
            else ra[i] = al.raw_unc(max(r, 0), ccol(c) * 8);
            aok |= (uint32_t)(r >= 0) << i;
        }
        if constexpr (EK == E_F32) {
            erow_nxt = ein ? erow_res : -1;
            const float* ax = (const float*)ep.d.aux + (long)max(erow_nxt, 0) * ep.d.ld + ecol;
#pragma unroll
            for (int i = 0; i < 4; ++i) aux_nxt[i] = *(const f32x4*)(ax + 4 * i);
        }
    };
    auto commit = [&]() {
#pragma unroll
        for (int i = 0; i < ACH; ++i) {
            const int c = tid + i * NTH;
            *(uint4*)(As + swzk(crow(c), ccol(c), K)) = ((aok >> i) & 1) ? al.cvt(ra[i]) : make_uint4(0, 0, 0, 0);
        }
    };
    const int G = gridDim.x;
    STAMP_DECL(8)
    auto tile_step = [&](int t) {
        STAMP_WAITV();
        STAMP(0);
        commit();
        if constexpr (EK == E_F32) {
            erow_cur = erow_nxt;
#pragma unroll
            for (int i = 0; i < 4; ++i) aux_cur[i] = aux_nxt[i];
        }
        STAMP(1);
        __syncthreads();
        STAMP(2);
        issue();
        resolve(t + 2 * G);
        STAMP(3);
        f32x4 acc[RT][CT];
#pragma unroll
        for (int i = 0; i < RT; ++i)
#pragma unroll
            for (int j = 0; j < CT; ++j) acc[i][j] = (f32x4){0.f, 0.f, 0.f, 0.f};
#pragma unroll
        for (int ks = 0; ks < K / 32; ++ks) {
            bf16x8 af[RT];
#pragma unroll
            for (int i = 0; i < RT; ++i) af[i] = *(const bf16x8*)(As + swzk(wr * 16 * RT + i * 16 + fr, ks * 4 + g, K));
#pragma unroll
            for (int j = 0; j < CT; ++j) {
                const bf16x8 bf = *(const bf16x8*)(Ws + swzk(wc * (N / 2) + j * 16 + fr, ks * 4 + g, K));
#pragma unroll
                for (int i = 0; i < RT; ++i) acc[i][j] = mfma32(af[i], bf, acc[i][j]);
            }
        }
        asm volatile("" :: "v"(acc[0][0][0]), "v"(acc[RT - 1][CT - 1][3]));
        STAMP(4);
        __syncthreads();
        STAMP(5);
        float* st = stage_all + wave * 16 * EP;
#pragma unroll
        for (int i = 0; i < RT; ++i)
#pragma unroll
            for (int j0 = 0; j0 < CT; j0 += 4) {
#pragma unroll
                for (int j = 0; j < 4; ++j)
#pragma unroll
                    for (int r = 0; r < 4; ++r) st[(4 * g + r) * EP + 16 * j + fr] = acc[i][j0 + j][r];
                const int m0 = t * BMT + wr * 16 * RT + i * 16, n0 = wc * (N / 2) + j0 * 16;
                if constexpr (EK == E_QKV_HEADS) {
                    const EpiDesc& d = ep.d;
                    const int h = d.p0, Lp = d.p2, L = d.p4;
                    const int r = lane & 15, slot = lane >> 4, nb = n0 + slot * 16, m = m0 + r;
                    if (m < d.M) {
                        const int ph = HS == 16 ? nb >> 4 : nb >> 5, lp = (h == 1) ? ph : fdiv(ph, h, d.mg1), hd = ph - lp * h;
                        const int part = lp + d.p1;
                        const int bw = fdiv(m, Lp, d.mg0), tt = m - bw * Lp;
                        const bool valid = tt < L;
                        float v[16];
                        float ss = 0.f;
#pragma unroll
                        for (int j = 0; j < 16; j += 4) {
                            const f32x4 x = *(const f32x4*)(st + r * EP + slot * 16 + j) + *(const f32x4*)(bs + nb + j);
#pragma unroll
                            for (int e = 0; e < 4; ++e) {
                                v[j + e] = valid ? x[e] : 0.f;
                                ss = fmaf(v[j + e], v[j + e], ss);
                            }
                        }
                        if constexpr (HS == 32) ss += __shfl_xor(ss, 16);
                        float rn = 1.f;
                        if (part < 2) {
                            rn = 1.f / fmaxf(sqrtf(ss), 1e-12f);
                            if (HS == 16 || !(slot & 1)) d.aux_out[(((long)bw * h + hd) * 2 + part) * Lp + tt] = valid ? rn : 0.f;
                        }
                        uint16_t* o = (uint16_t*)d.out + ((((long)bw * h + hd) * 3 + part) * Lp + tt) * HS + (HS == 32 ? (slot & 1) * 16 : 0);
                        float w8[8];
#pragma unroll
                        for (int e = 0; e < 8; ++e) w8[e] = v[e] * rn;
                        *(uint4*)o = pack8(w8);
#pragma unroll
                        for (int e = 0; e < 8; ++e) w8[e] = v[8 + e] * rn;
                        *(uint4*)(o + 8) = pack8(w8);
                    }
                } else if constexpr (EK == E_F32) {
                    if (erow_cur >= 0) {
                        float* o = (float*)ep.d.out + (long)erow_cur * ep.d.ld + ecol;
                        const int r = lane >> 2, c0 = (lane & 3) * 16;
#pragma unroll
                        for (int q = 0; q < 4; ++q)
                            *(f32x4*)(o + 4 * q) = *(const f32x4*)(st + r * EP + c0 + 4 * q) + *(const f32x4*)(bs + ecol + 4 * q) + aux_cur[q];
                    }
                } else {
                    ep.tile(st, m0, n0, lane);
                }
            }
        STAMP(6);
        __syncthreads();
        STAMP(7);
    };
    int t = blockIdx.x;
    resolve(t);
    issue();
    resolve(t + G);
#pragma unroll
    for (int i = 0; i < WCH; ++i) {
        const int c = tid + i * NTH, n = c / KC, kc = c - n * KC;
        *(uint4*)(Ws + swzk(n, kc, K)) = *(const uint4*)(Wb + (long)n * K + kc * 8);
    }

    STAMP_START();
    for (; t < ntiles; t += G) tile_step(t);
#ifdef SWV2_RW_STAMPS
    if (tid == 0)
        for (int k = 0; k < 8; ++k) rw_stamps[blockIdx.x * 8 + k] = st_acc[k];
#endif
}

enum class LinearKernel {
    RESIDENT_QKV128 = SWV2_LINEAR_RESIDENT_QKV128, RESIDENT_QKV192X3 = SWV2_LINEAR_RESIDENT_QKV192X3, RESIDENT_DX128 = SWV2_LINEAR_RESIDENT_DX128,
    WIDE_DMA = SWV2_LINEAR_WIDE_DMA, WIDE = SWV2_LINEAR_WIDE, TILE64 = SWV2_LINEAR_TILE64, TILE128 = SWV2_LINEAR_TILE128
};

constexpr bool qkv_pair(int ak, int ek) { return ak == A_F32 && ek == E_QKV_HEADS; }
constexpr bool dx_pair(int ak, int ek) { return ak == A_HEADS && ek == E_F32; }
constexpr bool loss_epi(int ek) { return ek == E_UNPATCH_LOSS || ek == E_UNPATCH_LOSS_SKIP; }
constexpr bool wide_pair(int ak, int ek) {
    return (ak == A_F32 || ak == A_BF16 || ak == A_HEADS) &&
           (ek == E_BF16 || ek == E_F32 || ek == E_F32_ACC || ek == E_QKV_HEADS || ek == E_HEADS || ek == E_GELU_GRAD || ek == E_BF16_GELU);
}
constexpr bool dma_loader(int ak) { return ak == A_BF16 || ak == A_HEADS; }

LinearKernel linear_kernel_for(int ak, int ek, const swv2_operand* a, const swv2_epilogue* e, int N, int wide) {
    const int M = a->rows, K = a->cols;
    if (qkv_pair(ak, ek) && M >= 256 * 128 && a->rowidx) {
        if (N == 384 && K == 128 && e->p[3] == 16) return LinearKernel::RESIDENT_QKV128;
        if (N == 768 && K == 192 && e->p[3] == 32 && e->p[0] == 8) return LinearKernel::RESIDENT_QKV192X3;
    }
    if (dx_pair(ak, ek) && N == 128 && K == 384 && M >= 256 * 64 && e->rowidx && e->aux && !a->rowidx) return LinearKernel::RESIDENT_DX128;
    if (wide_pair(ak, ek)) {
        const bool part192 = dx_pair(ak, ek) && N == 192 && K == 768 && !a->rowidx && M >= 64 * WBM &&
                             (double)a->rows * a->cols * 2 < 4.29e9;
        if (wide && (N % WBN == 0 || part192) && K % BK == 0 && (N >= 512 || part192) && K >= 512 && M >= 16 * WBM) {
            const bool small = (double)a->rows * (ak == A_HEADS ? a->cols : a->ld) * 2 < 4.29e9;
            return dma_loader(ak) && small && K % 128 == 0 && (ak == A_HEADS || !a->rowidx) ? LinearKernel::WIDE_DMA : LinearKernel::WIDE;
        }
    }
    if (loss_epi(ek)) return LinearKernel::TILE64;
    if (qkv_pair(ak, ek) || dx_pair(ak, ek)) {
        const double w1 = cdiv(M, BM), w2 = cdiv(M, BM / 2), slots = 768.0;
        const double e1 = w1 / (std::ceil(w1 / slots) * slots), e2 = w2 / (std::ceil(w2 / slots) * slots);
        if (e2 > e1 + 0.08) return LinearKernel::TILE64;
    }
    return LinearKernel::TILE128;
}

int linear_epi_kind(int ak, const swv2_epilogue* e) {
    static_assert(E_BF16 == SWV2_EPI_BF16 && E_BF16_GELU == SWV2_EPI_BF16_GELU && A_F32 == SWV2_OP_F32 && A_BF16_CS == SWV2_OP_BF16_CSCALE,
                  "A_* / E_* mirror the public kinds");
    if (ak == A_BF16_CS) {
        if (e->kind == SWV2_EPI_F32) return E_F32;
        swv2_set_error("swv2_linear: SWV2_OP_BF16_CSCALE supports SWV2_EPI_F32 only (got %d)", e->kind);
        return SWV2_ERR_INVALID;
    }
    if (ak == A_F32 && e->kind == SWV2_EPI_UNPATCH_LOSS) return e->p[3] ? E_UNPATCH_LOSS_SKIP : E_UNPATCH_LOSS;
    if (e->kind >= SWV2_EPI_BF16 && e->kind <= SWV2_EPI_BF16_GELU) return e->kind;
    swv2_set_error("swv2_linear: unknown epilogue kind %d (or not available for operand kind %d)", e->kind, ak);
    return SWV2_ERR_INVALID;
}

template <int EK>
Epi<EK> make_epi(const swv2_epilogue* e, int M, int N) {
    Epi<EK> ep;
    ep.d.out = e->out; ep.d.bias = e->bias; ep.d.aux = e->aux; ep.d.aux_out = e->aux_out; ep.d.rowidx = e->rowidx;
    ep.d.ld = e->ld; ep.d.M = M; ep.d.N = N;
    ep.d.p0 = e->p[0]; ep.d.p1 = e->p[1]; ep.d.p2 = e->p[2]; ep.d.p3 = e->p[3]; ep.d.p4 = e->p[4];
    ep.d.mg0 = ep.d.mg1 = ep.d.mg2 = 0;
    ep.d.loss_tar = nullptr; ep.d.loss_qw = nullptr; ep.d.loss_part = nullptr; ep.d.loss_resid = nullptr; ep.d.q0 = ep.d.q1 = ep.d.q2 = ep.d.q3 = 0;
    if (EK == E_QKV_HEADS || EK == E_HEADS) { ep.d.mg0 = fdiv_magic(e->p[2]); ep.d.mg1 = fdiv_magic(e->p[0]); ep.d.mg2 = fdiv_magic(e->p[3]); }
    if (EK == E_UNPATCH || loss_epi(EK)) { ep.d.mg0 = fdiv_magic((e->p[1] / 4) * (e->p[2] / 4)); ep.d.mg1 = fdiv_magic(e->p[2] / 4); }
    if (loss_epi(EK)) {
        ep.d.loss_tar = e->loss_tar; ep.d.loss_qw = e->loss_qw; ep.d.loss_part = e->loss_part; ep.d.loss_resid = (uint16_t*)e->loss_resid;
        ep.d.q0 = e->q[0]; ep.d.q1 = e->q[1];
        const long nb = M / ((e->p[1] / 4) * (e->p[2] / 4)), plane = (long)e->p[1] * e->p[2];
        ep.d.q2 = e->q[2] ? e->q[2] : (int)(nb * e->p[0] * plane);
        ep.d.q3 = (int)(nb * e->ld * plane);
    }
    return ep;
}

template <int AK, int EK>
int launch_nt2(const swv2_operand* a, const void* w, const swv2_epilogue* e, int M, int N, int K, hipStream_t st) {
    const Epi<EK> ep = make_epi<EK>(e, M, N);
    const uint16_t* wb = (const uint16_t*)w;
    const LinearKernel kern = linear_kernel_for(AK, EK, a, e, N, swv2_gemm_wide());
    switch (kern) {
        case LinearKernel::RESIDENT_QKV128:
            if constexpr (qkv_pair(AK, EK)) {
                Epi<EK> ep1 = ep;
                ep1.d.p1 = 0;
                hipLaunchKernelGGL((gemm_rw_kernel<AK, EK, 384, 128, 128>), dim3(256), dim3(512), 0, st, make_loader<AK>(a), wb, ep1, M);
            }
            break;
        case LinearKernel::RESIDENT_QKV192X3:
            if constexpr (qkv_pair(AK, EK)) {
                for (int part = 0; part < 3; ++part) {
                    Epi<EK> ep2 = ep;
                    ep2.d.N = 256;
                    ep2.d.p1 = part;
                    ep2.d.bias = e->bias ? e->bias + 256 * part : nullptr;
                    hipLaunchKernelGGL((gemm_rw_kernel<AK, EK, 256, 192, 128, 32>), dim3(256), dim3(512), 0, st, make_loader<AK>(a),
                                       wb + (size_t)part * 256 * 192, ep2, M);
                }
            }
            break;
        case LinearKernel::RESIDENT_DX128:
            if constexpr (dx_pair(AK, EK))
                hipLaunchKernelGGL((gemm_rw_kernel<AK, EK, 128, 384, 64>), dim3(256), dim3(512), 0, st, make_loader<AK>(a), wb, ep, M);
            break;
        case LinearKernel::WIDE_DMA:
        case LinearKernel::WIDE:
            if constexpr (wide_pair(AK, EK)) {
                SWV2_CHECK_ARG((double)N * K * 2 < 4.29e9, "swv2_linear: weight too large for the wide kernel's 32-bit offsets");
                const int mtiles = cdiv(M, WBM), ntn = cdiv(N, WBN), groups = cdiv(mtiles, 8);
                const int vmax = cdiv(groups, 8) * 8 * ntn;
                if (kern == LinearKernel::WIDE_DMA) {
                    if constexpr (dma_loader(AK))
                        hipLaunchKernelGGL((gemm_nt_wide_dma_kernel<AK, EK>), dim3(8 * (vmax < 32 || !swv2_wide_persist() ? vmax : 32)), dim3(WTH), 0, st,
                                           make_loader<AK>(a), wb, ep, M, N, K, mtiles, ntn, vmax);
                } else {
                    hipLaunchKernelGGL((gemm_nt_wide_kernel<AK, EK>), dim3(8 * vmax), dim3(WTH), 0, st, make_loader<AK>(a), wb, ep, M, N, K, mtiles, ntn);
                }
            }
            break;
        case LinearKernel::TILE64:
            if constexpr (qkv_pair(AK, EK) || dx_pair(AK, EK) || loss_epi(EK))
                hipLaunchKernelGGL((gemm_nt_kernel<AK, EK, BM / 2>), dim3(cdiv(M, BM / 2)), dim3(NTHREADS), 0, st, make_loader<AK>(a), wb, ep, M, N, K);
            break;
        case LinearKernel::TILE128:
            if constexpr (!loss_epi(EK))
                hipLaunchKernelGGL((gemm_nt_kernel<AK, EK>), dim3(cdiv(M, BM)), dim3(NTHREADS), 0, st, make_loader<AK>(a), wb, ep, M, N, K);
            break;
    }
    SWV2_CHECK_LAUNCH("swv2_linear");
    return SWV2_OK;
}

template <int AK>
int launch_nt1(const swv2_operand* a, const void* w, const swv2_epilogue* e, int M, int N, int K, hipStream_t st) {
    const int ek = linear_epi_kind(AK, e);
    if (ek < 0) return ek;
    if constexpr (AK == A_BF16_CS) {
        return launch_nt2<AK, E_F32>(a, w, e, M, N, K, st);
    } else {
    if constexpr (AK == A_F32) {
        if (ek == E_UNPATCH_LOSS_SKIP) return launch_nt2<AK, E_UNPATCH_LOSS_SKIP>(a, w, e, M, N, K, st);
        if (ek == E_UNPATCH_LOSS) return launch_nt2<AK, E_UNPATCH_LOSS>(a, w, e, M, N, K, st);
    }
    switch (ek) {
        case E_BF16: return launch_nt2<AK, E_BF16>(a, w, e, M, N, K, st);
        case E_F32: return launch_nt2<AK, E_F32>(a, w, e, M, N, K, st);
        case E_F32_ACC: return launch_nt2<AK, E_F32_ACC>(a, w, e, M, N, K, st);
        case E_QKV_HEADS: return launch_nt2<AK, E_QKV_HEADS>(a, w, e, M, N, K, st);
        case E_HEADS: return launch_nt2<AK, E_HEADS>(a, w, e, M, N, K, st);
        case E_GELU_GRAD: return launch_nt2<AK, E_GELU_GRAD>(a, w, e, M, N, K, st);
        case E_UNPATCH: return launch_nt2<AK, E_UNPATCH>(a, w, e, M, N, K, st);
        case E_BF16_GELU: return launch_nt2<AK, E_BF16_GELU>(a, w, e, M, N, K, st);
    }
    return SWV2_ERR_INVALID;
    }
}

}

int swv2_tn_wide_launch(const swv2_operand* y, const swv2_operand* x, float* part, float* dbpart, int M, int N, int K, int S, hipStream_t st) {
    const int tiles = (N / WBM) * (K / WBN), wgs = S * tiles, per_xcd = cdiv(wgs, 8);
#define SWV2_TNW(YK_, XK_)                                                                                                           \
    hipLaunchKernelGGL((gemm_tn_wide_kernel<YK_, XK_>), dim3(8 * per_xcd), dim3(WTH), 0, st, make_loader<YK_>(y), make_loader<XK_>(x), part, \
                       dbpart, M, N, K, S, wgs, per_xcd)
    if (y->kind == SWV2_OP_BF16 && x->kind == SWV2_OP_BF16) SWV2_TNW(A_BF16, A_BF16);
    else if (y->kind == SWV2_OP_BF16 && x->kind == SWV2_OP_HEADS) SWV2_TNW(A_BF16, A_HEADS);
    else if (y->kind == SWV2_OP_HEADS && x->kind == SWV2_OP_BF16) SWV2_TNW(A_HEADS, A_BF16);
    else { swv2_set_error("swv2_linear_wgrad: wide kernel: operand pair (%d, %d) not instantiated", y->kind, x->kind); return SWV2_ERR_UNSUPPORTED; }
#undef SWV2_TNW
    SWV2_CHECK_LAUNCH("swv2_linear_wgrad");
    return SWV2_OK;
}

#ifdef SWV2_RW_STAMPS
extern "C" int swv2_debug_rw_stamps(void* out) {
    return hipMemcpyFromSymbol(out, HIP_SYMBOL(rw_stamps), sizeof(unsigned long long) * 256 * 8) == hipSuccess ? 0 : -3;
}
#endif

extern "C" int swv2_linear_kernel(const swv2_operand* a, const swv2_epilogue* e, int N) {
    SWV2_CHECK_ARG(a && e && N > 0 && a->rows > 0 && a->cols > 0, "swv2_linear_kernel: null operand / epilogue or empty product");
    SWV2_CHECK_ARG(a->kind >= SWV2_OP_F32 && a->kind <= SWV2_OP_BF16_CSCALE, "swv2_linear_kernel: unknown operand kind %d", a->kind);
    const int ek = linear_epi_kind(a->kind, e);
    return ek < 0 ? ek : (int)linear_kernel_for(a->kind, ek, a, e, N, swv2_gemm_wide());
}

extern "C" int swv2_linear(const swv2_operand* a, const void* w_bf16, const swv2_epilogue* e, int N, void* stream) {
    int rc = check_operand(a, "swv2_linear");
    if (rc) return rc;
    SWV2_CHECK_ARG(w_bf16 && e && e->out && N > 0, "swv2_linear: null weight / epilogue / N");
    SWV2_CHECK_ARG(((uintptr_t)w_bf16 & 15) == 0 && ((uintptr_t)e->out & 15) == 0, "swv2_linear: unaligned pointer");
    if (e->kind == SWV2_EPI_BF16_GELU) SWV2_CHECK_ARG(e->aux_out != nullptr, "swv2_linear: GELU epilogue needs aux_out");
    if (e->kind == SWV2_EPI_BF16 || e->kind == SWV2_EPI_GELU_GRAD || e->kind == SWV2_EPI_BF16_GELU)
        SWV2_CHECK_ARG(e->ld % 8 == 0 && e->ld >= N, "swv2_linear: output pitch %ld must be a multiple of 8 and >= N", e->ld);
    if (e->kind == SWV2_EPI_F32 || e->kind == SWV2_EPI_F32_ACC)
        SWV2_CHECK_ARG(e->ld % 4 == 0 && e->ld >= N, "swv2_linear: output pitch %ld must be a multiple of 4 and >= N", e->ld);
    if (e->kind == SWV2_EPI_QKV_HEADS || e->kind == SWV2_EPI_HEADS)
        SWV2_CHECK_ARG((e->p[3] == 16 || e->p[3] == 32 || e->p[3] == 64 || e->p[3] == 96 || e->p[3] == 128 || e->p[3] == 256) && N % e->p[3] == 0 && e->p[0] > 0 && e->p[2] > 0,
                       "swv2_linear: head-split epilogue needs DP in {16,32,64,96,128,256} and N a multiple of DP (DP=%d N=%d)", e->p[3], N);
    if (e->kind == SWV2_EPI_UNPATCH || e->kind == SWV2_EPI_UNPATCH_LOSS)
        SWV2_CHECK_ARG(N == e->p[0] * 16, "swv2_linear: un-patchify needs N == Cout*16");
    if (e->kind == SWV2_EPI_UNPATCH_LOSS) {
        SWV2_CHECK_ARG(a->kind == SWV2_OP_F32, "swv2_linear: the loss epilogue takes an fp32 operand");
        SWV2_CHECK_ARG((e->p[4] == 0 || (e->p[4] >= e->p[0] && e->q[2] > 0)) && (!e->aux_out || e->ld >= e->p[0]) && e->q[2] >= 0,
                       "swv2_linear: loss epilogue: p[4] (channels of the destination tensor) needs q[2] (its dump offset), aux_out needs ld >= Cout");
        SWV2_CHECK_ARG(e->loss_tar && e->loss_qw && e->loss_part && e->loss_resid && e->q[0] >= e->q[1] + e->p[0] && e->q[1] >= 0,
                       "swv2_linear: the loss epilogue needs target, quadrature weights, sums, residual and q[1] + Cout <= q[0]");
        SWV2_CHECK_ARG((((uintptr_t)e->loss_tar | (uintptr_t)e->loss_resid) & 15) == 0, "swv2_linear: unaligned loss pointer");
        const double plane_ = (double)e->p[1] * e->p[2], nb_ = (double)a->rows / ((e->p[1] / 4) * (e->p[2] / 4));
        SWV2_CHECK_ARG((e->p[1] / 4) * (e->p[2] / 4) >= SWV2_LOSS_GROUP_ROWS, "swv2_linear: the loss epilogue needs at least %d patches per sample", SWV2_LOSS_GROUP_ROWS);
        const double cmax_ = fmax(fmax((double)e->p[3], (double)e->p[0]), fmax((double)e->p[4], e->aux_out ? (double)e->ld : 0.0));
        SWV2_CHECK_ARG(nb_ * e->q[0] * plane_ < 4.29e9 && nb_ * cmax_ * plane_ + 1024 < 4.29e9 && (double)a->rows * SWV2_LOSS_RESID_PITCH(N) + 2048 < 4.29e9 && (double)e->q[2] < 4.29e9,
                       "swv2_linear: the loss epilogue indexes its tensors with 32-bit element offsets (tensor too large)");
    }
    const int M = a->rows, K = a->cols;
    hipStream_t st = (hipStream_t)stream;
    switch (a->kind) {
        case SWV2_OP_F32: return launch_nt1<A_F32>(a, w_bf16, e, M, N, K, st);
        case SWV2_OP_BF16: return launch_nt1<A_BF16>(a, w_bf16, e, M, N, K, st);
        case SWV2_OP_BF16_GELU: return launch_nt1<A_BF16_GELU>(a, w_bf16, e, M, N, K, st);
        case SWV2_OP_HEADS: return launch_nt1<A_HEADS>(a, w_bf16, e, M, N, K, st);
        case SWV2_OP_PATCH: return launch_nt1<A_PATCH>(a, w_bf16, e, M, N, K, st);
        case SWV2_OP_MERGE_LN: return launch_nt1<A_MERGE_LN>(a, w_bf16, e, M, N, K, st);
        case SWV2_OP_BF16_CSCALE: return launch_nt1<A_BF16_CS>(a, w_bf16, e, M, N, K, st);
    }
    swv2_set_error("swv2_linear: unknown operand kind %d", a->kind);
    return SWV2_ERR_INVALID;
}
```

swin_v2_weather_amd/ops.py:

```python
from __future__ import annotations

import ctypes as C
import functools
from typing import Optional

import torch

from . import _lib as L

BF16 = torch.bfloat16


def _p(t: Optional[torch.Tensor]):
    return None if t is None else t.data_ptr()


def _stream():
    return torch.cuda.current_stream().cuda_stream


_TIMED = None


_EVERY = 1
_EVPOOL = []


def prewarm_events(n):
    for _ in range(n):
        a, b = torch.cuda.Event(enable_timing=True), torch.cuda.Event(enable_timing=True)
        a.record(); b.record()
        _EVPOOL.append((a, b))


def _event_pair():
    if _EVPOOL:
        return _EVPOOL.pop()
    a, b = torch.cuda.Event(enable_timing=True), torch.cuda.Event(enable_timing=True)
    a.record(); b.record()
    return a, b


def start_kernel_timing(names, every=1):
    global _TIMED, _EVERY
    _TIMED = {n: [] for n in names}
    _EVERY = max(1, int(every))
    _RR["fwd"] = _RR["bwd"] = 0


def stop_kernel_timing():
    global _TIMED
    rec, _TIMED = _TIMED, None
    torch.cuda.synchronize()
    out = {n: (len(ev), sum(a.elapsed_time(b) for a, b in ev) / max(len(ev), 1)) for n, ev in (rec or {}).items()}
    for ev in (rec or {}).values():
        _EVPOOL.extend(ev)
    return out


BLOCK_KERNEL_IDS = {"qkv": 1, "attn_fwd": 2, "proj": 3, "ln1_fwd": 4, "fc1": 5, "fc2": 6, "ln2_fwd": 7, "ln2_bwd": 11,
                    "wgrad_fc2": 12, "dh": 13, "wgrad_fc1": 14, "dx1": 15, "ln1_bwd": 16, "wgrad_proj": 17, "doh": 18,
                    "attn_bwd": 19, "wgrad_qkv": 20, "dx": 21,
                    "proj_ln_fwd": 3, "mlp_fwd": 5, "mlp_bwd": 13, "proj_ln_bwd": 16,
                    "wgrad_group": 22}


_RR = {"fwd": 0, "bwd": 0}


def block_event_pair(phase, desc):
    desc.ev_kernel = 0
    rec = _TIMED
    if rec is None:
        return
    mine = [n for n in rec if BLOCK_KERNEL_IDS.get(n, 0) and ((BLOCK_KERNEL_IDS[n] < 10) == (phase == "fwd"))]
    if not mine:
        return
    turn = _RR[phase]
    _RR[phase] += 1
    if turn % _EVERY:
        return
    n = mine[(turn // _EVERY) % len(mine)]
    a, b = _event_pair()
    desc.ev_kernel, desc.ev_start, desc.ev_stop = BLOCK_KERNEL_IDS[n], a.cuda_event, b.cuda_event
    rec[n].append((a, b))


def _timed(name, fn, *args):
    rec = _TIMED
    if rec is None or name not in rec:
        return fn(*args)
    a, b = _event_pair()
    a.record()
    r = fn(*args)
    b.record()
    rec[name].append((a, b))
    return r


def _chk(t: torch.Tensor, dtype, name: str):
    if t.dtype != dtype or not t.is_contiguous() or not t.is_cuda:
        raise L.Swv2Error(f"{name}: expected a contiguous CUDA {dtype} tensor, got {t.dtype} "
                          f"contiguous={t.is_contiguous()} device={t.device}")
    return t


def attn_geometry(Lwin: int, head_dim: int):
    lp, dp = C.c_int(), C.c_int()
    L.check(L.load().swv2_attn_geometry(Lwin, head_dim, C.byref(lp), C.byref(dp)), "swv2_attn_geometry")
    return lp.value, dp.value


def operand(kind, t, rows, cols, ld=0, rowidx=None, aux=(None, None, None, None), p=(0, 0, 0, 0)) -> L.Operand:
    o = L.Operand()
    o.kind, o.ptr, o.rowidx = kind, _p(t), _p(rowidx)
    o.aux0, o.aux1, o.aux2, o.aux3 = (_p(a) for a in aux)
    o.ld, o.rows, o.cols = ld, rows, cols
    o.p = (C.c_int * 4)(*p)
    o._keep = (t, rowidx, aux)
    return o


def op_f32(x2d: torch.Tensor, rows=None, rowidx=None):
    _chk(x2d, torch.float32, "op_f32")
    return operand(L.OP_F32, x2d, rows if rows is not None else x2d.shape[0], x2d.shape[1], x2d.shape[1], rowidx)


def op_bf16(x2d: torch.Tensor, rows=None, rowidx=None, gelu=False):
    _chk(x2d, BF16, "op_bf16")
    return operand(L.OP_BF16_GELU if gelu else L.OP_BF16, x2d, rows if rows is not None else x2d.shape[0],
                   x2d.shape[1], x2d.shape[1], rowidx)


def op_bf16_cscale(x2d: torch.Tensor, coef: torch.Tensor, rows_per_sample: int, cols: int = 0):
    _chk(x2d, BF16, "op_bf16_cscale"); _chk(coef, torch.float32, "op_bf16_cscale coef")
    cols = cols or x2d.shape[1]
    if coef.dim() != 2 or coef.shape[1] * 16 != cols or coef.shape[0] * rows_per_sample != x2d.shape[0] or cols > x2d.shape[1]:
        raise L.Swv2Error(f"op_bf16_cscale: coef {tuple(coef.shape)} does not match rows {x2d.shape[0]} / {rows_per_sample}, cols {cols}")
    return operand(L.OP_BF16_CSCALE, x2d, x2d.shape[0], cols, x2d.shape[1], aux=(coef, None, None, None),
                   p=(rows_per_sample, 0, coef.shape[1], 0))


def op_heads(t: torch.Tensor, Bw, heads, parts, Lp, DP):
    _chk(t, BF16, "op_heads")
    return operand(L.OP_HEADS, t, Bw * Lp, parts * heads * DP, parts, p=(heads, 0, Lp, DP))


def op_patch(x4d: torch.Tensor):
    _chk(x4d, torch.float32, "op_patch")
    B, Cin, H, W = x4d.shape
    return operand(L.OP_PATCH, x4d, B * (H // 4) * (W // 4), Cin * 16, 0, p=(Cin, H, W, 0))


def op_merge_ln(x4d, mean, rstd, gamma, beta):
    B, H, W, Cc = x4d.shape
    return operand(L.OP_MERGE_LN, x4d, B * (H // 2) * (W // 2), 4 * Cc, 0, aux=(mean, rstd, gamma, beta), p=(H, W, Cc, 0))


def epilogue(kind, out, ld=0, bias=None, aux=None, aux_out=None, rowidx=None, p=(0, 0, 0, 0, 0), loss=None) -> L.Epilogue:
    e = L.Epilogue()
    e.kind, e.out, e.bias, e.aux, e.aux_out, e.rowidx, e.ld = kind, _p(out), _p(bias), _p(aux), _p(aux_out), _p(rowidx), ld
    e.p = (C.c_int * 5)(*p)
    e._keep = (out, bias, aux, aux_out, rowidx, loss)
    if loss is not None:
        tar, qw, part, resid, coff = loss[:5]
        base = loss[5] if len(loss) > 5 else None
        _chk(tar, torch.float32, "loss target"); _chk(qw, torch.float32, "quadrature weights")
        _chk(resid, BF16, "loss residual"); _chk(part, torch.float32, "loss partial sums")
        if resid.dim() != 2 or resid.shape[1] % 64:
            raise L.Swv2Error(f"loss epilogue: residual rows must be padded to whole 128-byte lines (ops._lib.loss_resid_pitch), got {tuple(resid.shape)}")
        behind = [(out if base is None else base, "out"), (resid, "residual")] + ([(aux_out, "second destination")] if aux_out is not None else [])
        for t_, nm in behind:
            room = t_.untyped_storage().nbytes() - (t_.storage_offset() + t_.numel()) * t_.element_size()
            if room < L.LOSS_DUMP_BYTES:
                raise L.Swv2Error(f"loss epilogue: {nm} needs {L.LOSS_DUMP_BYTES} bytes of allocated scratch behind it ({room} found)")
        e.loss_tar, e.loss_qw, e.loss_part, e.loss_resid = _p(tar), _p(qw), _p(part), _p(resid)
        dump = 0
        if base is not None:
            dump = (base.data_ptr() + base.numel() * 4 - out.data_ptr()) // 4
        e.q = (C.c_int * 3)(tar.shape[1], coff, dump)
    return e


def linear(a: L.Operand, w_bf16: torch.Tensor, e: L.Epilogue, N: int, tag: str = "linear"):
    _chk(w_bf16, BF16, "linear weight")
    if w_bf16.shape[0] != N or w_bf16.shape[1] != a.cols:
        raise L.Swv2Error(f"linear: weight {tuple(w_bf16.shape)} does not match N={N} K={a.cols}")
    L.check(_timed(tag, L.load().swv2_linear, C.byref(a), _p(w_bf16), C.byref(e), N, _stream()), "swv2_linear")


def linear_wgrad(dy: L.Operand, x: L.Operand, dW: torch.Tensor, db: Optional[torch.Tensor], nmap=None, kmap=None,
                 splits: int = 0, workspace: bool = True):
    _chk(dW, torch.float32, "dW")
    ldw = dW.shape[-1] if dW.dim() == 2 else dW[0].numel()
    lib = L.load()
    if splits <= 0:
        tiles = ((dy.cols + 127) // 128) * ((x.cols + 127) // 128)
        splits = max(8, (512 // tiles) // 8 * 8)
        if tiles < 3:
            splits = max(8, splits // 16 * 8)
    if not workspace:
        L.check(lib.swv2_linear_wgrad(C.byref(dy), C.byref(x), _p(dW), _p(db), _p(nmap), _p(kmap), ldw, splits, _stream()),
                "swv2_linear_wgrad")
        return
    nbytes = lib.swv2_linear_wgrad_ws_bytes(dy.rows, dy.cols, x.cols, splits)
    ws = torch.empty(nbytes, dtype=torch.uint8, device=dW.device)
    L.check(lib.swv2_linear_wgrad_ws(C.byref(dy), C.byref(x), _p(dW), _p(db), _p(nmap), _p(kmap), ldw, splits, _p(ws), nbytes,
                                     _stream()), "swv2_linear_wgrad_ws")


def prep_weight(w: torch.Tensor, transpose=False, row_map=None, out_rows=None, col_map=None, out_cols=None):
    w2 = w.detach().reshape(w.shape[0], -1)
    _chk(w2, torch.float32, "prep_weight")
    rows, cols = w2.shape
    r_t, c_t = (cols, rows) if transpose else (rows, cols)
    out_rows = out_rows if out_rows is not None else r_t
    out_cols = out_cols if out_cols is not None else c_t
    out = torch.empty(out_rows, out_cols, dtype=BF16, device=w.device)
    L.check(L.load().swv2_prep_weight(_p(w2), rows, cols, int(transpose), _p(row_map), out_rows, _p(col_map), out_cols,
                                      _p(out), _stream()), "swv2_prep_weight")
    return out


class PrepBatch:

    _tables = {}

    def __init__(self):
        self.jobs, self.keep, self.done = [], [], []

    def on_launched(self, fn):
        self.done.append(fn)

    def add(self, w: torch.Tensor, transpose=False, row_map=None, out_rows=None, col_map=None, out_cols=None, out=None, f32=False):
        w2 = w.detach().reshape(w.shape[0], -1)
        _chk(w2, torch.float32, "PrepBatch.add")
        rows, cols = w2.shape
        r_t, c_t = (cols, rows) if transpose else (rows, cols)
        out_rows = out_rows if out_rows is not None else r_t
        out_cols = out_cols if out_cols is not None else c_t
        dt = torch.float32 if f32 else BF16
        if out is None or out.dtype != dt or tuple(out.shape) != (out_rows, out_cols) or out.device != w.device or not out.is_contiguous():
            out = torch.empty(out_rows, out_cols, dtype=dt, device=w.device)
        self.jobs.append((_p(w2), rows, cols, int(transpose), _p(row_map), out_rows, _p(col_map), out_cols, _p(out), int(f32)))
        self.keep.append((w2, row_map, col_map, out))
        return out

    def launch(self):
        if not self.jobs:
            for fn in self.done:
                fn()
            self.done = []
            return
        lib = L.load()
        key = tuple(self.jobs)
        t = PrepBatch._tables.get(key)
        dev = self.keep[0][3].device
        if t is None:
            arr = (L.PrepItem * len(self.jobs))()
            pairs = []
            for i, j in enumerate(self.jobs):
                arr[i] = L.PrepItem(*j)
                pairs += [(i, c) for c in range(lib.swv2_prep_item_chunks(j[5], j[7], j[3]))]
            host = torch.frombuffer(bytearray(bytes(arr)), dtype=torch.uint8).clone()
            t = (host.to(dev), torch.tensor(pairs, dtype=torch.int32).to(dev), len(pairs))
            if len(PrepBatch._tables) > 64:
                PrepBatch._tables.clear()
            PrepBatch._tables[key] = t
        L.check(lib.swv2_prep_multi(_p(t[0]), _p(t[1]), t[2], _stream()), "swv2_prep_multi")
        for fn in self.done:
            fn()
        self.jobs, self.keep, self.done = [], [], []


def ln_residual_fwd(a, res, gamma, beta, scale, rowidx, y, mean, rstd, M, Cc, res_mod, rows_per_sample, eps=1e-5):
    g = L.LnArgs()
    g.a, g.res, g.gamma, g.beta, g.scale, g.rowidx = _p(a), _p(res), _p(gamma), _p(beta), _p(scale), _p(rowidx)
    g.y, g.mean, g.rstd = _p(y), _p(mean), _p(rstd)
    g.M, g.C, g.res_mod, g.rows_per_sample, g.eps = M, Cc, res_mod, rows_per_sample, eps
    L.check(L.load().swv2_ln_residual_fwd(C.byref(g), _stream()), "swv2_ln_residual_fwd")


def ln_residual_bwd(a, dy, gamma, scale, rowidx, mean, rstd, da, dgamma, dbeta, M, Cc, rows_per_sample):
    g = L.LnArgs()
    g.a, g.dy, g.gamma, g.scale, g.rowidx = _p(a), _p(dy), _p(gamma), _p(scale), _p(rowidx)
    g.mean, g.rstd, g.da, g.dgamma, g.dbeta = _p(mean), _p(rstd), _p(da), _p(dgamma), _p(dbeta)
    ws = torch.empty(L.LN_BWD_MAX_BLOCKS * 2 * Cc, dtype=torch.float32, device=a.device)
    g.ws = _p(ws)
    g.M, g.C, g.res_mod, g.rows_per_sample, g.eps = M, Cc, 0, rows_per_sample, 1e-5
    L.check(L.load().swv2_ln_residual_bwd(C.byref(g), _stream()), "swv2_ln_residual_bwd")


def attn_args(qkvh, logit_scale, bias, oh, lse, Bw, heads, Lwin, head_dim, nwh, nww, mask_thr, doh=None, rnorm=None,
              dqkvh=None, dlogit=None, dbias=None, max_chunks=64, bias_pack=None, dbias_ws=None) -> L.AttnArgs:
    a = L.AttnArgs()
    a.qkvh, a.logit_scale, a.bias, a.oh, a.lse = _p(qkvh), _p(logit_scale), _p(bias), _p(oh), _p(lse)
    a.bias_pack = _p(bias_pack)
    a.doh, a.rnorm, a.dqkvh, a.dlogit_scale, a.dbias = _p(doh), _p(rnorm), _p(dqkvh), _p(dlogit), _p(dbias)
    a.Bw, a.heads, a.L, a.head_dim, a.nwh, a.nww, a.mask_thr, a.max_chunks = Bw, heads, Lwin, head_dim, nwh, nww, mask_thr, max_chunks
    if dbias_ws is not None:
        a.dbias_ws, a.dbias_ws_bytes = _p(dbias_ws), dbias_ws.numel() * dbias_ws.element_size()
    return a


def attn_pack_bias(bias: torch.Tensor) -> torch.Tensor:
    heads, Lw = bias.shape[0], bias.shape[1]
    out = torch.empty(L.load().swv2_attn_pack_bias_bytes(heads, Lw), dtype=torch.uint8, device=bias.device)
    L.check(L.load().swv2_attn_pack_bias(_p(bias), heads, Lw, _p(out), _stream()), "swv2_attn_pack_bias")
    return out


def attn_fwd(a: L.AttnArgs):
    L.check(_timed("attn_fwd", L.load().swv2_attn_fwd, C.byref(a), _stream()), "swv2_attn_fwd")


def attn_bwd(a: L.AttnArgs):
    L.check(_timed("attn_bwd", L.load().swv2_attn_bwd, C.byref(a), _stream()), "swv2_attn_bwd")


def batch_sum(inp: torch.Tensor, out: torch.Tensor, accumulate=False):
    B = inp.shape[0]
    n = inp[0].numel()
    L.check(L.load().swv2_batch_sum(_p(inp), _p(out), B, n, int(accumulate), _stream()), "swv2_batch_sum")


def merge_stats(x, mean, rstd, eps=1e-5):
    B, H, W, Cc = x.shape
    L.check(L.load().swv2_merge_stats(_p(x), _p(mean), _p(rstd), B, H, W, Cc, eps, _stream()), "swv2_merge_stats")


def merge_ln_bwd(x, dn, gamma, mean, rstd, dx, dgamma, dbeta):
    B, H, W, Cc = x.shape
    L.check(L.load().swv2_merge_ln_bwd(_p(x), _p(dn), _p(gamma), _p(mean), _p(rstd), _p(dx), _p(dgamma), _p(dbeta),
                                       B, H, W, Cc, _stream()), "swv2_merge_ln_bwd")


def loss_sums(prd, tar, qw, sums, ws=None):
    B, Cc, H, W = prd.shape
    if ws is None:
        ws = loss_workspace(B * Cc, H, W, prd.device)
    L.check(L.load().swv2_loss_sums(_p(prd), _p(tar), _p(qw), _p(sums), B * Cc, H, W, _p(ws), ws.numel() * 4, _stream()), "swv2_loss_sums")


def loss_finalize(sums, chw, absolute: bool, squared: bool, loss, coef):
    layers = sums.shape[0] if sums.dim() == 4 else 1
    BC, Cc = sums.shape[-3] * sums.shape[-2], chw.numel()
    L.check(L.load().swv2_loss_finalize(_p(sums), layers, _p(chw), BC, Cc, int(absolute), int(squared), _p(loss), _p(coef), _stream()),
            "swv2_loss_finalize")


def loss_part_reduce(part, M, T, B, Cout, coff, sums):
    L.check(L.load().swv2_loss_part_reduce(_p(part), M, T, B, Cout, sums.shape[2], coff, _p(sums), _stream()), "swv2_loss_part_reduce")


def loss_resid_to_image(resid, coef, out, Cout: int, add=None):
    _chk(resid, BF16, "loss residual"); _chk(coef, torch.float32, "coef"); _chk(out, torch.float32, "out")
    B, Cs, H, W = out.shape
    if resid.shape[1] != L.loss_resid_pitch(Cout * 16):
        raise L.Swv2Error(f"loss_resid_to_image: residual rows of {resid.shape[1]} elements, expected the padded pitch {L.loss_resid_pitch(Cout * 16)}")
    if add is not None:
        _chk(add, torch.float32, "add")
    L.check(L.load().swv2_loss_resid_to_image(_p(resid), _p(coef), _p(add), _p(out), B, Cout, H, W, Cs, add.shape[1] if add is not None else 0,
                                              _stream()), "swv2_loss_resid_to_image")


def loss_finalize_sums(sums, chw, absolute: bool, squared: bool):
    B, Cc = sums.shape[-3:-1]
    buf = torch.empty(B * Cc + 1, dtype=torch.float32, device=sums.device)
    coef, loss = buf[:B * Cc].view(B, Cc), buf[B * Cc:]
    loss_finalize(sums, chw, absolute, squared, loss, coef)
    return loss, coef


def loss_grad(prd, tar, qw, coef, dprd):
    B, Cc, H, W = prd.shape
    L.check(L.load().swv2_loss_grad(_p(prd), _p(tar), _p(qw), _p(coef), _p(dprd), B * Cc, H, W, _stream()), "swv2_loss_grad")


def score_slices(planes: int, H: int, W: int) -> int:
    return int(L.load().swv2_score_slices(planes, H, W))


def score_workspace(planes: int, H: int, W: int, device) -> torch.Tensor:
    return torch.empty(int(L.load().swv2_score_ws_bytes(planes, H, W)) // 4, dtype=torch.float32, device=device)


def _planes_in_place(t: torch.Tensor, lead: int) -> bool:
    if not (t.is_cuda and t.dtype == torch.float32 and t.dim() == lead + 3 and t.numel() > 0):
        return False
    B, (Cc, H, W), bs = t.shape[lead - 1], t.shape[lead:], t.stride(lead - 1)
    return tuple(t.stride()[lead:]) == (H * W, W, 1) and t.data_ptr() % 16 == 0 and (B == 1 or (bs % 4 == 0 and bs >= Cc * H * W))


def score_planes_ok(t: torch.Tensor) -> bool:
    return _planes_in_place(t, 1) and t.shape[3] % 4 == 0


def score_sums(prd, tar, w, ws, clim=None):
    if not (score_planes_ok(prd) and score_planes_ok(tar)) or prd.shape != tar.shape:
        raise L.Swv2Error(f"score_sums: expected two CUDA fp32 [B, C, H, W] tensors of one shape with contiguous planes and W % 4 == 0, got "
                          f"{tuple(prd.shape)} {prd.dtype} strides {prd.stride()} / {tuple(tar.shape)} {tar.dtype} strides {tar.stride()}")
    B, Cc, H, W = prd.shape
    _chk(w, torch.float32, "row weights"); _chk(ws, torch.float32, "score workspace")
    if w.numel() != H:
        raise L.Swv2Error(f"score_sums: {w.numel()} row weights for {H} rows")
    if clim is not None and (_chk(clim, torch.float32, "climatology").shape != (Cc, H, W)):
        raise L.Swv2Error(f"score_sums: climatology {tuple(clim.shape)}, expected {(Cc, H, W)}")
    L.check(L.load().swv2_score_sums(_p(prd), prd.stride(0) if B > 1 else Cc * H * W, _p(tar), tar.stride(0) if B > 1 else Cc * H * W,
                                     _p(clim), _p(w), B, Cc, H, W, _p(ws), ws.numel() * 4, _stream()), "swv2_score_sums")


def score_finalize(ws, B: int, Cc: int, H: int, W: int, scale=None):
    _chk(ws, torch.float32, "score workspace")
    if scale is not None and _chk(scale, torch.float32, "scale").numel() != Cc:
        raise L.Swv2Error(f"score_finalize: scale of {scale.numel()} values for {Cc} channels")
    n = B * Cc
    buf = torch.empty(6 * n + 2 * Cc, dtype=torch.float32, device=ws.device)
    sums, rmse, acc = buf[:4 * n].view(B, Cc, 4), buf[4 * n:5 * n].view(B, Cc), buf[5 * n:6 * n].view(B, Cc)
    rmse_mean, acc_mean = buf[6 * n:6 * n + Cc], buf[6 * n + Cc:]
    L.check(L.load().swv2_score_finalize(_p(ws), ws.numel() * 4, B, Cc, H, W, _p(scale), _p(sums), _p(rmse), _p(acc), _p(rmse_mean),
                                         _p(acc_mean), _stream()), "swv2_score_finalize")
    return sums, rmse, acc, rmse_mean, acc_mean


def forecast_scores(prd, tar, w, clim=None, scale=None, ws=None):
    B, Cc, H, W = prd.shape
    if ws is None:
        ws = score_workspace(B * Cc, H, W, prd.device)
    score_sums(prd, tar, w, ws, clim)
    return score_finalize(ws, B, Cc, H, W, scale)


def l1_workspace(planes: int, H: int, W: int, device) -> torch.Tensor:
    return torch.empty(int(L.load().swv2_l1_ws_bytes(planes, H, W)) // 4, dtype=torch.float32, device=device)


def loss_workspace(planes: int, H: int, W: int, device) -> torch.Tensor:
    return torch.empty(int(L.load().swv2_loss_ws_bytes(planes, H, W)) // 4, dtype=torch.float32, device=device)


def l1_sums(prd, tar, w, ws):
    if not (score_planes_ok(prd) and score_planes_ok(tar)) or prd.shape != tar.shape:
        raise L.Swv2Error(f"l1_sums: expected two CUDA fp32 [B, C, H, W] tensors of one shape with contiguous planes and W % 4 == 0, got "
                          f"{tuple(prd.shape)} {prd.dtype} strides {prd.stride()} / {tuple(tar.shape)} {tar.dtype} strides {tar.stride()}")
    B, Cc, H, W = prd.shape
    _chk(w, torch.float32, "row weights"); _chk(ws, torch.float32, "l1 workspace")
    if w.numel() != H:
        raise L.Swv2Error(f"l1_sums: {w.numel()} row weights for {H} rows")
    L.check(L.load().swv2_l1_sums(_p(prd), prd.stride(0) if B > 1 else Cc * H * W, _p(tar), tar.stride(0) if B > 1 else Cc * H * W, _p(w),
                                  B, Cc, H, W, _p(ws), ws.numel() * 4, _stream()), "swv2_l1_sums")


def l1_finalize(ws, B: int, Cc: int, H: int, W: int, chw=None, absolute: bool = False):
    _chk(ws, torch.float32, "l1 workspace")
    if chw is not None and _chk(chw, torch.float32, "channel weights").numel() != Cc:
        raise L.Swv2Error(f"l1_finalize: {chw.numel()} channel weights for {Cc} channels")
    n = B * Cc
    buf = torch.empty(3 * n + 2, dtype=torch.float32, device=ws.device)
    sums = buf[:2 * n].view(B, Cc, 2)
    coef, loss = (buf[2 * n:3 * n].view(B, Cc), buf[3 * n:3 * n + 1]) if chw is not None else (None, None)
    L.check(L.load().swv2_l1_finalize(_p(ws), ws.numel() * 4, B, Cc, H, W, _p(chw), int(absolute), _p(sums), _p(loss), _p(coef), _stream()),
            "swv2_l1_finalize")
    return sums, loss, coef


def l1_grad(prd, tar, qw, coef, dprd):
    for t, what in ((prd, "prediction"), (tar, "target"), (dprd, "gradient"), (qw, "row weights"), (coef, "coef")):
        _chk(t, torch.float32, what)
    B, Cc, H, W = prd.shape
    if tar.shape != prd.shape or dprd.shape != prd.shape or coef.numel() != B * Cc or qw.numel() != H:
        raise L.Swv2Error(f"l1_grad: shapes {tuple(prd.shape)} / {tuple(tar.shape)} / {tuple(dprd.shape)}, coef {coef.numel()}, weights {qw.numel()}")
    L.check(L.load().swv2_l1_grad(_p(prd), _p(tar), _p(qw), _p(coef), _p(dprd), B * Cc, H, W, _stream()), "swv2_l1_grad")


def sht_power(table, X, keep_coeffs: bool = False, zero_coeffs: bool = False):
    _chk(table, torch.float32, "sht table"); _chk(X, torch.float32, "sht operand")
    if table.dim() != 3 or X.dim() != 3 or X.shape[0] != table.shape[0] or X.shape[2] != table.shape[2] or X.shape[1] % 2:
        raise L.Swv2Error(f"sht_power: table {tuple(table.shape)} [mmax, lmax, nlat] against operand {tuple(X.shape)} [mmax, 2 planes, nlat]")
    mmax, lmax, nlat = table.shape
    planes = X.shape[1] // 2
    lib = L.load()
    nb = lib.swv2_sht_ws_bytes(planes, lmax, mmax)
    ws = _scratch(nb, X.device, "sht_power")
    power = torch.empty(planes, lmax, dtype=torch.float32, device=X.device)
    coef = (torch.zeros if zero_coeffs else torch.empty)(mmax, 2 * planes, lmax, dtype=torch.float32, device=X.device) if keep_coeffs else None
    L.check(_timed("sht_power", lib.swv2_sht_power, _p(table), _p(X), _p(power), _p(coef), planes, nlat, lmax, mmax, _p(ws), nb, _stream()),
            "swv2_sht_power")
    return power, coef


def sht_repack(src, planes: int, nlat: int, mmax: int, scale: float, backward: bool = False):
# ... 385 lines not shown
```

Baseline: 225.5.

## Add compact row walk to resident QKV/DX GEMMs skipping window padding rows

Adds a compact row-walk mode to the resident-weight QKV and dX GEMM kernels. Rows are mapped through the window padding (L valid of Lp), so padded rows are never computed. In the QKV case the padded output slots are zeroed explicitly instead. The block code now builds the qkv/dx products with operand p[1]/p[2] set whenever L < Lp, so the default swv2_linear path can pick the compact walk when the shape matches. The cost is extra index arithmetic (a magic division per row) and a separate zero-fill loop in the epilogue.

```diff
diff --git a/include/swv2.h b/include/swv2.h
--- a/include/swv2.h
+++ b/include/swv2.h
@@ -142,6 +142,11 @@
 #define SWV2_LINEAR_TILE64 5
 #define SWV2_LINEAR_TILE128 6
 int swv2_linear_kernel(const swv2_operand* a, const swv2_epilogue* e, int N);
+
+#define SWV2_ROW_WALK_PADDED 0
+#define SWV2_ROW_WALK_COMPACT 1
+int swv2_linear_row_walk(const swv2_operand* a, const swv2_epilogue* e, int N);
+int swv2_linear_resident(const swv2_operand* a, const void* w_bf16, const swv2_epilogue* e, int N, int row_walk, void* stream);
 
 int swv2_linear_wgrad(const swv2_operand* dy, const swv2_operand* x, float* dW, float* db, const int32_t* nmap,
                       const int32_t* kmap, int ldw, int splits, void* stream);
@@ -492,6 +497,8 @@
 int swv2_block_step_id(int step);
 const char* swv2_block_step_name(int step);
 
+int swv2_block_row_walk(const swv2_block_desc* d, int step);
+
 int swv2_block_fwd(const swv2_block_desc* d, void* stream);
 int swv2_block_bwd(const swv2_block_desc* d, void* stream);
 
diff --git a/swin_v2_weather_amd/_lib.py b/swin_v2_weather_amd/_lib.py
--- a/swin_v2_weather_amd/_lib.py
+++ b/swin_v2_weather_amd/_lib.py
@@ -198,6 +198,7 @@
 EPI_BF16, EPI_F32, EPI_QKV_HEADS, EPI_GELU_GRAD, EPI_UNPATCH, EPI_HEADS, EPI_F32_ACC, EPI_BF16_GELU, EPI_UNPATCH_LOSS = range(9)
 LINEAR_RESIDENT_QKV128, LINEAR_RESIDENT_QKV192X3, LINEAR_RESIDENT_DX128, LINEAR_WIDE_DMA, LINEAR_WIDE, LINEAR_TILE64, LINEAR_TILE128 = range(7)
 LINEAR_WIDE_KERNELS, LINEAR_TILE_KERNELS = (LINEAR_WIDE_DMA, LINEAR_WIDE), (LINEAR_TILE64, LINEAR_TILE128)
+ROW_WALK_PADDED, ROW_WALK_COMPACT = range(2)
 WGRAD_WIDE, WGRAD_TILE = range(2)
 BLOCK_WGRAD_SLAB, BLOCK_WGRAD_GROUPED = range(2)
 
@@ -218,6 +219,9 @@
     "swv2_attn_bwd": (_I, [C.POINTER(AttnArgs), _P]),
     "swv2_linear": (_I, [C.POINTER(Operand), _P, C.POINTER(Epilogue), _I, _P]),
     "swv2_linear_kernel": (_I, [C.POINTER(Operand), C.POINTER(Epilogue), _I]),
+    "swv2_linear_row_walk": (_I, [C.POINTER(Operand), C.POINTER(Epilogue), _I]),
+    "swv2_linear_resident": (_I, [C.POINTER(Operand), _P, C.POINTER(Epilogue), _I, _I, _P]),
+    "swv2_block_row_walk": (_I, [C.POINTER(BlockDesc), _I]),
     "swv2_linear_wgrad_kernel": (_I, [C.POINTER(Operand), C.POINTER(Operand), _I, C.c_size_t]),
     "swv2_block_wgrad_kernel": (_I, [C.POINTER(WgradItem), _I, C.c_size_t]),
     "swv2_linear_wgrad": (_I, [C.POINTER(Operand), C.POINTER(Operand), _P, _P, _P, _P, _I, _I, _P]),
diff --git a/swin_v2_weather_amd/csrc/block.hip b/swin_v2_weather_amd/csrc/block.hip
--- a/swin_v2_weather_amd/csrc/block.hip
+++ b/swin_v2_weather_amd/csrc/block.hip
@@ -37,6 +37,20 @@
     it[2].dW = d->d_proj_w; it[2].db = d->d_proj_b; it[2].kmap = d->proj_map; it[2].ldw = C;
     it[3].dy = op_heads(d->dqkvh, Bw, h, 3, d->Lp, d->DP); it[3].x = op(SWV2_OP_F32, d->x, Mw, C, C, d->rowidx);
     it[3].dW = d->d_qkv_w; it[3].db = d->d_qkv_b; it[3].nmap = d->qkv_map; it[3].ldw = C;
+}
+struct product { swv2_operand a; swv2_epilogue e; int N; };
+product qkv_product(const swv2_block_desc* d) {
+    const int Mw = d->B * d->nwh * d->nww * d->Lp, h = d->heads;
+    product q = {op(SWV2_OP_F32, d->x, Mw, d->C, d->C, d->rowidx), epi(SWV2_EPI_QKV_HEADS, d->qkvh, 0, d->qkv_b_pad, nullptr, d->rnorm), 3 * h * d->DP};
+    q.e.p[0] = h; q.e.p[2] = d->Lp; q.e.p[3] = d->DP; q.e.p[4] = d->L;
+    if (d->L < d->Lp) { q.a.p[1] = d->L; q.a.p[2] = d->Lp; }
+    return q;
+}
+product dx_product(const swv2_block_desc* d) {
+    const int Bw = d->B * d->nwh * d->nww;
+    product q = {op_heads(d->dqkvh, Bw, d->heads, 3, d->Lp, d->DP), epi(SWV2_EPI_F32, d->dx, d->C, nullptr, d->dx1, nullptr, d->rowidx), d->C};
+    if (d->L < d->Lp) { q.e.p[2] = d->Lp; q.e.p[4] = d->L; }
+    return q;
 }
 #define TRY(x) do { int rc_ = (x); if (rc_) return rc_; } while (0)
 
@@ -134,6 +148,13 @@
     return SWV2_OK;
 }
 
+extern "C" int swv2_block_row_walk(const swv2_block_desc* d, int step) {
+    SWV2_CHECK_ARG(d && (step == SWV2_STEP_QKV || step == SWV2_STEP_DX), "swv2_block_row_walk: null descriptor, or a step that is neither the qkv nor the dx product");
+    SWV2_CHECK_ARG(d->B > 0 && d->C > 0 && d->heads > 0 && d->Lp > 0 && d->DP > 0 && d->nwh > 0 && d->nww > 0, "swv2_block_row_walk: non-positive geometry");
+    const product q = step == SWV2_STEP_QKV ? qkv_product(d) : dx_product(d);
+    return swv2_linear_row_walk(&q.a, &q.e, q.N);
+}
+
 extern "C" int swv2_block_fwd(const swv2_block_desc* d, void* st) {
     SWV2_CHECK_ARG(d && d->x && d->x2 && d->qkvh && d->rowidx, "swv2_block_fwd: null descriptor field");
     swv2_block_plan_t p;
@@ -148,10 +169,8 @@
         }
         break;
     case SWV2_STEP_QKV: {
-        swv2_operand a = op(SWV2_OP_F32, d->x, Mw, C, C, d->rowidx);
-        swv2_epilogue e = epi(SWV2_EPI_QKV_HEADS, d->qkvh, 0, d->qkv_b_pad, nullptr, d->rnorm);
-        e.p[0] = h; e.p[2] = d->Lp; e.p[3] = d->DP; e.p[4] = d->L;
-        LAUNCH(SWV2_STEP_QKV, swv2_linear(&a, d->w_qkv, &e, 3 * h * d->DP, st));
+        const product q = qkv_product(d);
+        LAUNCH(SWV2_STEP_QKV, swv2_linear(&q.a, d->w_qkv, &q.e, q.N, st));
     } break;
     case SWV2_STEP_QK_NORMALIZE: TRY(swv2_qk_normalize(d->qkvh, (float*)d->rnorm, Bw, h, d->Lp, d->L, d->DP, st)); break;
     case SWV2_STEP_PACK_BIAS: TRY(swv2_attn_pack_bias(d->bias, h, d->L, d->bias_pack, st)); break;
@@ -269,8 +288,8 @@
         LAUNCH(SWV2_STEP_ATTN_BWD, swv2_attn_bwd(&a, st));
     } break;
     case SWV2_STEP_DX: {
-        swv2_epilogue e = epi(SWV2_EPI_F32, d->dx, C, nullptr, d->dx1, nullptr, d->rowidx);
-        LAUNCH(SWV2_STEP_DX, swv2_linear(&it[3].dy, d->w_qkvt, &e, C, st));
+        const product q = dx_product(d);
+        LAUNCH(SWV2_STEP_DX, swv2_linear(&q.a, d->w_qkvt, &q.e, q.N, st));
     } break;
     case SWV2_STEP_LN_FOLD:
         swv2_launch_ln_partials_reduce2(d->ln_ws, d->d_n2_w, d->d_n2_b, n_ln2, ln1_ws, d->d_n1_w, d->d_n1_b, n_ln1, C, (hipStream_t)st);
diff --git a/swin_v2_weather_amd/csrc/gemm.hip b/swin_v2_weather_amd/csrc/gemm.hip
--- a/swin_v2_weather_amd/csrc/gemm.hip
+++ b/swin_v2_weather_amd/csrc/gemm.hip
@@ -964,8 +964,10 @@
 #include "stamps.h"
 __device__ __forceinline__ int swzk(int r, int kc, int K) { return r * K + ((kc ^ ((r >> 1) & 7)) << 3); }
 
-template <int AK, int EK, int N, int K, int BMT, int HS = 16>
-__global__ __launch_bounds__(512) void gemm_rw_kernel(ALoad<AK> al, const uint16_t* __restrict__ Wb, Epi<EK> ep, int M) {
+struct RowWalk { int L, Lp; uint32_t mgL; };
+
+template <int AK, int EK, int N, int K, int BMT, int HS = 16, bool CW = false>
+__global__ __launch_bounds__(512) void gemm_rw_kernel(ALoad<AK> al, const uint16_t* __restrict__ Wb, Epi<EK> ep, int M, RowWalk rwk) {
     constexpr int NTH = 512, KC = K / 8;
     constexpr int ACH = BMT * KC / NTH;
     constexpr int RT = BMT / 64;
@@ -1000,6 +1002,10 @@
     uint32_t ain = 0;
     uint32_t aok = 0;
     bool ein = false;
+    auto wrow = [&](int m) {
+        if constexpr (CW) return m + fdiv(m, rwk.L, rwk.mgL) * (rwk.Lp - rwk.L);
+        else return m;
+    };
     auto resolve = [&](int t) {
         ain = 0;
 #pragma unroll
@@ -1007,13 +1013,13 @@
             const int c = tid + i * NTH, m = t * BMT + crow(c);
             const bool in = (t < ntiles) && (m < M);
             ain |= (uint32_t)in << i;
-            if constexpr (AK == A_F32) arow[i] = al.d.rowidx[min(m, M - 1)];
-            else arow[i] = min(m, M - 1);
+            if constexpr (AK == A_F32) arow[i] = al.d.rowidx[wrow(min(m, M - 1))];
+            else arow[i] = wrow(min(m, M - 1));
         }
         if constexpr (EK == E_F32) {
             const int m = t * BMT + wr * 16 + (lane >> 2);
             ein = (t < ntiles) && (m < M);
-            erow_res = ein ? ep.d.rowidx[m] : -1;
+            erow_res = ein ? ep.d.rowidx[wrow(m)] : -1;
         }
     };
     auto issue = [&]() {
@@ -1092,11 +1098,11 @@
                     const EpiDesc& d = ep.d;
                     const int h = d.p0, Lp = d.p2, L = d.p4;
                     const int r = lane & 15, slot = lane >> 4, nb = n0 + slot * 16, m = m0 + r;
-                    if (m < d.M) {
+                    if (m < M) {
                         const int ph = HS == 16 ? nb >> 4 : nb >> 5, lp = (h == 1) ? ph : fdiv(ph, h, d.mg1), hd = ph - lp * h;
                         const int part = lp + d.p1;
-                        const int bw = fdiv(m, Lp, d.mg0), tt = m - bw * Lp;
-                        const bool valid = tt < L;
+                        const int bw = CW ? fdiv(m, L, rwk.mgL) : fdiv(m, Lp, d.mg0), tt = m - bw * (CW ? L : Lp);
+                        const bool valid = CW || tt < L;
                         float v[16];
                         float ss = 0.f;
 #pragma unroll
@@ -1135,6 +1141,21 @@
                     ep.tile(st, m0, n0, lane);
                 }
             }
+        if constexpr (CW && EK == E_QKV_HEADS) {
+            const EpiDesc& d = ep.d;
+            const int h = d.p0, Lp = d.p2, L = d.p4, per = (Lp - L) * (HS / 8);
+            const int w_end = fdiv(min(t * BMT + BMT, M), L, rwk.mgL);
+            for (int w = fdiv(t * BMT, L, rwk.mgL); w < w_end; ++w) {
+                for (int sl = tid >> 5; sl < 3 * h; sl += NTH / 32) {
+                    uint4* o = (uint4*)((uint16_t*)d.out + (((long)w * 3 * h + sl) * Lp + L) * HS);
+                    for (int j = tid & 31; j < per; j += 32) o[j] = make_uint4(0, 0, 0, 0);
+                }
+                for (int sl = tid >> 5; sl < 2 * h; sl += NTH / 32) {
+                    float* o = d.aux_out + ((long)w * 2 * h + sl) * Lp + L;
+                    for (int j = tid & 31; j < Lp - L; j += 32) o[j] = 0.f;
+                }
+            }
+        }
         STAMP(6);
         __syncthreads();
         STAMP(7);
@@ -1171,13 +1192,13 @@
 }
 constexpr bool dma_loader(int ak) { return ak == A_BF16 || ak == A_HEADS; }
 
-LinearKernel linear_kernel_for(int ak, int ek, const swv2_operand* a, const swv2_epilogue* e, int N, int wide) {
+LinearKernel linear_kernel_for(int ak, int ek, const swv2_operand* a, const swv2_epilogue* e, int N, int wide, bool any_rows = false) {
     const int M = a->rows, K = a->cols;
-    if (qkv_pair(ak, ek) && M >= 256 * 128 && a->rowidx) {
+    if (qkv_pair(ak, ek) && (M >= 256 * 128 || any_rows) && a->rowidx) {
         if (N == 384 && K == 128 && e->p[3] == 16) return LinearKernel::RESIDENT_QKV128;
         if (N == 768 && K == 192 && e->p[3] == 32 && e->p[0] == 8) return LinearKernel::RESIDENT_QKV192X3;
     }
-    if (dx_pair(ak, ek) && N == 128 && K == 384 && M >= 256 * 64 && e->rowidx && e->aux && !a->rowidx) return LinearKernel::RESIDENT_DX128;
+    if (dx_pair(ak, ek) && N == 128 && K == 384 && (M >= 256 * 64 || any_rows) && e->rowidx && e->aux && !a->rowidx) return LinearKernel::RESIDENT_DX128;
     if (wide_pair(ak, ek)) {
         const bool part192 = dx_pair(ak, ek) && N == 192 && K == 768 && !a->rowidx && M >= 64 * WBM &&
                              (double)a->rows * a->cols * 2 < 4.29e9;
@@ -1193,6 +1214,13 @@
         if (e2 > e1 + 0.08) return LinearKernel::TILE64;
     }
     return LinearKernel::TILE128;
+}
+
+int row_walk_for(LinearKernel kern, const swv2_operand* a, const swv2_epilogue* e, int N) {
+    int L = 0, Lp = 0;
+    if (kern == LinearKernel::RESIDENT_QKV128 && a->p[1] == e->p[4] && a->p[2] == e->p[2] && N == 3 * e->p[0] * e->p[3]) { L = e->p[4]; Lp = e->p[2]; }
+    if (kern == LinearKernel::RESIDENT_DX128 && e->p[2] == a->p[2]) { L = e->p[4]; Lp = a->p[2]; }
+    return L >= 2 && L < Lp && a->rows % Lp == 0 ? L : 0;
 }
 
 int linear_epi_kind(int ak, const swv2_epilogue* e) {
@@ -1230,16 +1258,31 @@
 }
 
 template <int AK, int EK>
-int launch_nt2(const swv2_operand* a, const void* w, const swv2_epilogue* e, int M, int N, int K, hipStream_t st) {
+int launch_nt2(const swv2_operand* a, const void* w, const swv2_epilogue* e, int M, int N, int K, hipStream_t st, int walk) {
     const Epi<EK> ep = make_epi<EK>(e, M, N);
     const uint16_t* wb = (const uint16_t*)w;
-    const LinearKernel kern = linear_kernel_for(AK, EK, a, e, N, swv2_gemm_wide());
+    const LinearKernel kern = linear_kernel_for(AK, EK, a, e, N, swv2_gemm_wide(), walk >= 0);
+    const int Lc = walk == SWV2_ROW_WALK_PADDED ? 0 : row_walk_for(kern, a, e, N);
+    if (walk >= 0) {
+        const bool resident = kern == LinearKernel::RESIDENT_QKV128 || kern == LinearKernel::RESIDENT_QKV192X3 || kern == LinearKernel::RESIDENT_DX128;
+        if (!resident || (walk == SWV2_ROW_WALK_COMPACT && !Lc)) {
+            swv2_set_error(!resident ? "swv2_linear_resident: no resident-weight kernel serves this product"
+                                     : "swv2_linear_resident: the compact walk needs the window-order promise (L, Lp) at a shape it is instantiated for");
+            return SWV2_ERR_UNSUPPORTED;
+        }
+    }
+    RowWalk rwk = {0, 0, 0u};
+    if (Lc) {
+        rwk.L = Lc; rwk.Lp = kern == LinearKernel::RESIDENT_DX128 ? a->p[2] : e->p[2]; rwk.mgL = fdiv_magic(Lc);
+    }
+    const int Mc = Lc ? M / rwk.Lp * Lc : M;
     switch (kern) {
         case LinearKernel::RESIDENT_QKV128:
             if constexpr (qkv_pair(AK, EK)) {
                 Epi<EK> ep1 = ep;
                 ep1.d.p1 = 0;
-                hipLaunchKernelGGL((gemm_rw_kernel<AK, EK, 384, 128, 128>), dim3(256), dim3(512), 0, st, make_loader<AK>(a), wb, ep1, M);
+                if (Lc) hipLaunchKernelGGL((gemm_rw_kernel<AK, EK, 384, 128, 128, 16, true>), dim3(256), dim3(512), 0, st, make_loader<AK>(a), wb, ep1, Mc, rwk);
+                else hipLaunchKernelGGL((gemm_rw_kernel<AK, EK, 384, 128, 128>), dim3(256), dim3(512), 0, st, make_loader<AK>(a), wb, ep1, M, rwk);
             }
             break;
         case LinearKernel::RESIDENT_QKV192X3:
@@ -1250,13 +1293,15 @@
                     ep2.d.p1 = part;
                     ep2.d.bias = e->bias ? e->bias + 256 * part : nullptr;
                     hipLaunchKernelGGL((gemm_rw_kernel<AK, EK, 256, 192, 128, 32>), dim3(256), dim3(512), 0, st, make_loader<AK>(a),
-                                       wb + (size_t)part * 256 * 192, ep2, M);
+                                       wb + (size_t)part * 256 * 192, ep2, M, rwk);
                 }
             }
             break;
         case LinearKernel::RESIDENT_DX128:
-            if constexpr (dx_pair(AK, EK))
-                hipLaunchKernelGGL((gemm_rw_kernel<AK, EK, 128, 384, 64>), dim3(256), dim3(512), 0, st, make_loader<AK>(a), wb, ep, M);
+            if constexpr (dx_pair(AK, EK)) {
+                if (Lc) hipLaunchKernelGGL((gemm_rw_kernel<AK, EK, 128, 384, 64, 16, true>), dim3(256), dim3(512), 0, st, make_loader<AK>(a), wb, ep, Mc, rwk);
+                else hipLaunchKernelGGL((gemm_rw_kernel<AK, EK, 128, 384, 64>), dim3(256), dim3(512), 0, st, make_loader<AK>(a), wb, ep, M, rwk);
+            }
             break;
         case LinearKernel::WIDE_DMA:
         case LinearKernel::WIDE:
@@ -1287,25 +1332,25 @@
 }
 
 template <int AK>
-int launch_nt1(const swv2_operand* a, const void* w, const swv2_epilogue* e, int M, int N, int K, hipStream_t st) {
+int launch_nt1(const swv2_operand* a, const void* w, const swv2_epilogue* e, int M, int N, int K, hipStream_t st, int walk) {
     const int ek = linear_epi_kind(AK, e);
     if (ek < 0) return ek;
     if constexpr (AK == A_BF16_CS) {
-        return launch_nt2<AK, E_F32>(a, w, e, M, N, K, st);
+        return launch_nt2<AK, E_F32>(a, w, e, M, N, K, st, walk);
     } else {
     if constexpr (AK == A_F32) {
-        if (ek == E_UNPATCH_LOSS_SKIP) return launch_nt2<AK, E_UNPATCH_LOSS_SKIP>(a, w, e, M, N, K, st);
-        if (ek == E_UNPATCH_LOSS) return launch_nt2<AK, E_UNPATCH_LOSS>(a, w, e, M, N, K, st);
+        if (ek == E_UNPATCH_LOSS_SKIP) return launch_nt2<AK, E_UNPATCH_LOSS_SKIP>(a, w, e, M, N, K, st, walk);
+        if (ek == E_UNPATCH_LOSS) return launch_nt2<AK, E_UNPATCH_LOSS>(a, w, e, M, N, K, st, walk);
     }
     switch (ek) {
-        case E_BF16: return launch_nt2<AK, E_BF16>(a, w, e, M, N, K, st);
-        case E_F32: return launch_nt2<AK, E_F32>(a, w, e, M, N, K, st);
-        case E_F32_ACC: return launch_nt2<AK, E_F32_ACC>(a, w, e, M, N, K, st);
-        case E_QKV_HEADS: return launch_nt2<AK, E_QKV_HEADS>(a, w, e, M, N, K, st);
-        case E_HEADS: return launch_nt2<AK, E_HEADS>(a, w, e, M, N, K, st);
-        case E_GELU_GRAD: return launch_nt2<AK, E_GELU_GRAD>(a, w, e, M, N, K, st);
-        case E_UNPATCH: return launch_nt2<AK, E_UNPATCH>(a, w, e, M, N, K, st);
-        case E_BF16_GELU: return launch_nt2<AK, E_BF16_GELU>(a, w, e, M, N, K, st);
+        case E_BF16: return launch_nt2<AK, E_BF16>(a, w, e, M, N, K, st, walk);
+        case E_F32: return launch_nt2<AK, E_F32>(a, w, e, M, N, K, st, walk);
+        case E_F32_ACC: return launch_nt2<AK, E_F32_ACC>(a, w, e, M, N, K, st, walk);
+        case E_QKV_HEADS: return launch_nt2<AK, E_QKV_HEADS>(a, w, e, M, N, K, st, walk);
+        case E_HEADS: return launch_nt2<AK, E_HEADS>(a, w, e, M, N, K, st, walk);
+        case E_GELU_GRAD: return launch_nt2<AK, E_GELU_GRAD>(a, w, e, M, N, K, st, walk);
+        case E_UNPATCH: return launch_nt2<AK, E_UNPATCH>(a, w, e, M, N, K, st, walk);
+        case E_BF16_GELU: return launch_nt2<AK, E_BF16_GELU>(a, w, e, M, N, K, st, walk);
     }
     return SWV2_ERR_INVALID;
     }
@@ -1340,7 +1385,12 @@
     return ek < 0 ? ek : (int)linear_kernel_for(a->kind, ek, a, e, N, swv2_gemm_wide());
 }
 
-extern "C" int swv2_linear(const swv2_operand* a, const void* w_bf16, const swv2_epilogue* e, int N, void* stream) {
+extern "C" int swv2_linear_row_walk(const swv2_operand* a, const swv2_epilogue* e, int N) {
+    const int kern = swv2_linear_kernel(a, e, N);
+    return kern < 0 ? kern : row_walk_for((LinearKernel)kern, a, e, N) ? SWV2_ROW_WALK_COMPACT : SWV2_ROW_WALK_PADDED;
+}
+
+static int linear_launch(const swv2_operand* a, const void* w_bf16, const swv2_epilogue* e, int N, void* stream, int walk) {
     int rc = check_operand(a, "swv2_linear");
     if (rc) return rc;
     SWV2_CHECK_ARG(w_bf16 && e && e->out && N > 0, "swv2_linear: null weight / epilogue / N");
@@ -1371,14 +1421,25 @@
     const int M = a->rows, K = a->cols;
     hipStream_t st = (hipStream_t)stream;
     switch (a->kind) {
-        case SWV2_OP_F32: return launch_nt1<A_F32>(a, w_bf16, e, M, N, K, st);
-        case SWV2_OP_BF16: return launch_nt1<A_BF16>(a, w_bf16, e, M, N, K, st);
-        case SWV2_OP_BF16_GELU: return launch_nt1<A_BF16_GELU>(a, w_bf16, e, M, N, K, st);
-        case SWV2_OP_HEADS: return launch_nt1<A_HEADS>(a, w_bf16, e, M, N, K, st);
-        case SWV2_OP_PATCH: return launch_nt1<A_PATCH>(a, w_bf16, e, M, N, K, st);
-        case SWV2_OP_MERGE_LN: return launch_nt1<A_MERGE_LN>(a, w_bf16, e, M, N, K, st);
-        case SWV2_OP_BF16_CSCALE: return launch_nt1<A_BF16_CS>(a, w_bf16, e, M, N, K, st);
+        case SWV2_OP_F32: return launch_nt1<A_F32>(a, w_bf16, e, M, N, K, st, walk);
+        case SWV2_OP_BF16: return launch_nt1<A_BF16>(a, w_bf16, e, M, N, K, st, walk);
+        case SWV2_OP_BF16_GELU: return launch_nt1<A_BF16_GELU>(a, w_bf16, e, M, N, K, st, walk);
+        case SWV2_OP_HEADS: return launch_nt1<A_HEADS>(a, w_bf16, e, M, N, K, st, walk);
+        case SWV2_OP_PATCH: return launch_nt1<A_PATCH>(a, w_bf16, e, M, N, K, st, walk);
+        case SWV2_OP_MERGE_LN: return launch_nt1<A_MERGE_LN>(a, w_bf16, e, M, N, K, st, walk);
+        case SWV2_OP_BF16_CSCALE: return launch_nt1<A_BF16_CS>(a, w_bf16, e, M, N, K, st, walk);
     }
     swv2_set_error("swv2_linear: unknown operand kind %d", a->kind);
     return SWV2_ERR_INVALID;
 }
+
+
+extern "C" int swv2_linear(const swv2_operand* a, const void* w_bf16, const swv2_epilogue* e, int N, void* stream) {
+    return linear_launch(a, w_bf16, e, N, stream, -1);
+}
+
+extern "C" int swv2_linear_resident(const swv2_operand* a, const void* w_bf16, const swv2_epilogue* e, int N, int row_walk, void* stream) {
+    SWV2_CHECK_ARG(row_walk == SWV2_ROW_WALK_PADDED || row_walk == SWV2_ROW_WALK_COMPACT, "swv2_linear_resident: unknown row walk %d", row_walk);
+    SWV2_CHECK_ARG(!e || e->kind != SWV2_EPI_QKV_HEADS || e->aux_out, "swv2_linear_resident: the qkv epilogue needs aux_out (rnorm)");
+    return linear_launch(a, w_bf16, e, N, stream, row_walk);
+}
diff --git a/swin_v2_weather_amd/ops.py b/swin_v2_weather_amd/ops.py
--- a/swin_v2_weather_amd/ops.py
+++ b/swin_v2_weather_amd/ops.py
@@ -187,6 +187,13 @@
     if w_bf16.shape[0] != N or w_bf16.shape[1] != a.cols:
         raise L.Swv2Error(f"linear: weight {tuple(w_bf16.shape)} does not match N={N} K={a.cols}")
     L.check(_timed(tag, L.load().swv2_linear, C.byref(a), _p(w_bf16), C.byref(e), N, _stream()), "swv2_linear")
+
+
+def linear_resident(a: L.Operand, w_bf16: torch.Tensor, e: L.Epilogue, N: int, row_walk: int):
+    _chk(w_bf16, BF16, "linear weight")
+    if w_bf16.shape[0] != N or w_bf16.shape[1] != a.cols:
+        raise L.Swv2Error(f"linear_resident: weight {tuple(w_bf16.shape)} does not match N={N} K={a.cols}")
+    L.check(L.load().swv2_linear_resident(C.byref(a), _p(w_bf16), C.byref(e), N, row_walk, _stream()), "swv2_linear_resident")
 
 
 def linear_wgrad(dy: L.Operand, x: L.Operand, dW: torch.Tensor, db: Optional[torch.Tensor], nmap=None, kmap=None,
```

Measured after the change: 226.8 (median of 6 runs). About the same (+0.5%).
